# santi-pdp/segan_pytorch

Hardware: AMD Instinct MI355X
Metric: 16384-sample waveform chunks/sec (GAN step) (higher is better)
Workload: dtype f32

## Files before the change

### include/segan_hip.h

```cpp
#ifndef SEGAN_HIP_H
#define SEGAN_HIP_H

#include <stddef.h>
#include <stdint.h>

#ifdef __cplusplus
extern "C" {
#endif

#define SEGAN_ABI_VERSION 16

#define SEGAN_PAD_REFLECT 0
#define SEGAN_PAD_ZERO 1

#define SEGAN_ACT_NONE 0
#define SEGAN_ACT_TANH 1

typedef struct segan_src {
  const float* p0;
  const float* p1;
  int32_t C0;
  int32_t C1;
  const float* scale;
  const float* shift;
  const float* slope;
} segan_src;

int segan_abi_version(void);
const char* segan_last_error(void);

int segan_set_reserved_slots(int n);

size_t segan_packed_f_bytes(int M, int N, int S);
size_t segan_packed_t_bytes(int M, int N, int S);

int segan_pack_weights(const float* w, float* wf, float* wt, int M, int N, int K, int S,
                       int pad_t, void* stream);

#define SEGAN_PREC_FP32 0
#define SEGAN_PREC_BF16 1
#define SEGAN_PREC_BF16X3 3
#define SEGAN_PREC_FP32_BLOCKED 4
size_t segan_packed_bf_bytes(int M, int N, int S, int tform, int planes);
int segan_pack_weights_bf(const float* w, void* out, int M, int N, int K, int S, int tform,
                          int pad_t, int planes, void* stream);

size_t segan_bf16_scratch_bytes(int op, int B, int N, int M, int L, int K, int S, int pad, int planes);
size_t segan_corr_scratch_bytes(void);
void segan_debug_last_corr(int* out6);
void segan_debug_last_wgrad(int* out6);

int segan_conv1d_fwd(const segan_src* x, const void* wf, const float* bias, float* out, int B,
                     int N, int M, int L, int K, int S, int padL, int mode, int roll,
                     int precision, void* scratch, size_t scratch_bytes, void* stream);

int segan_conv1d_dgrad(const float* da, const void* wt, const float* w, float* dx, float* halo,
                       int B, int N, int M, int L, int K, int S, int padL, int roll, int precision,
                       void* scratch, size_t scratch_bytes, void* stream);

#define SEGAN_WGRAD_DETERMINISTIC 1
size_t segan_wgrad_scratch_bytes(int B, int M, int N, int Ls, int S, int precision, int flags);
int segan_wgrad(const segan_src* lo, const segan_src* hi, float* dw, int B, int M, int N, int Ls,
                int K, int S, int padL, int mode, int roll, int precision, int flags, void* scratch,
                size_t scratch_bytes, void* stream);

int segan_deconv1d_fwd(const segan_src* x, const void* wt, const float* w, const float* bias,
                       float* y, int B, int M, int N, int Ls, int K, int S, int pad, int act,
                       int precision, void* scratch, size_t scratch_bytes, void* stream);

int segan_deconv1d_dgrad(const float* dy, const void* wf, float* dx0, float* dx1, int B, int M,
                         int M0, int N, int Ls, int K, int S, int pad, int precision, void* scratch,
                         size_t scratch_bytes, void* stream);


int segan_bn_nsplit(int B, int C, int L);
int segan_bn_stats(const float* x, const float* gamma, const float* beta, float eps,
                   float momentum, float* running_mean, float* running_var, float* mean,
                   float* rstd, float* scale, float* shift, float* ws, int B, int C, int L,
                   void* stream);
int segan_bn_partial(const float* x, float* ws, int B, int C, int L, void* stream);
int segan_bn_final(const float* ws, int nsplit_total, const float* gamma, const float* beta,
                   float eps, float momentum, float* running_mean, float* running_var, float* mean,
                   float* rstd, float* scale, float* shift, int C, void* stream);

int segan_affine_tanh(const float* x, const float* scale, const float* shift, float* y, int B,
                      int C, int L, void* stream);
int segan_scale_mask(const float* x, const float* scale, const float* mask, float* y, int B, int C,
                     int L, void* stream);

int segan_affine_prelu(const float* x, const float* scale, const float* shift, const float* slope,
                       float* y, int B, int C, int L, void* stream);

int segan_sum_skip(const float* x0, const float* slope0, const float* x1, const float* alpha,
                   float* out, int B, int C, int L, void* stream);

int segan_act_bwd(const float* a, const float* dh, const float* dskip, const float* slope,
                  const float* alpha, const float* bn_mean, const float* bn_rstd,
                  const float* bn_gamma, const float* bn_beta, float* da, float* dslope,
                  float* dalpha, float* dgamma, float* dbeta, float* dbias, float* ws, int B, int C,
                  int L, void* stream);
int segan_act_bwd_bn_reduce(const float* a, const float* dh, const float* slope,
                            const float* bn_mean, const float* bn_rstd, const float* bn_gamma,
                            const float* bn_beta, float* dslope, float* dgamma, float* dbeta,
                            float* totals, float* ws, int B, int C, int L, void* stream);
int segan_act_bwd_bn_apply(const float* a, const float* dh, const float* slope,
                           const float* bn_mean, const float* bn_rstd, const float* bn_gamma,
                           const float* bn_beta, const float* totals, float* da, float* dbias,
                           float* ws, int B, int C, int L, double count_total, void* stream);

int segan_tanh_bwd(const float* y, const float* dy, const float* clean, float l1_scale, float* da,
                   float* dbias, float* ws, int B, int C, int L, void* stream);


#define SEGAN_GEMM_DETERMINISTIC 1
size_t segan_gemm_scratch_bytes(int M, int N, int K);
int segan_gemm(const float* A, int64_t sam, int64_t sak, const float* B, int64_t sbk, int64_t sbn,
               float* C, int64_t ldc, int M, int N, int K, int beta0, int flags, void* scratch,
               size_t scratch_bytes, void* stream);

int segan_bias_prelu_rows(const float* x, const float* bias, const float* slope, float* y,
                          int rows, int cols, void* stream);
int segan_bias_prelu_rows_bwd(const float* x, const float* bias, const float* slope,
                              const float* dy, float* dx, float* dslope, float* dbias, int rows,
                              int cols, void* stream);

int segan_mse_const(const float* x, float target, float* loss, float* grad, const float* gout,
                    float gscale, int n, void* stream);
int segan_bce_logits_const(const float* x, float target, float* loss, float* grad,
                           const float* gout, float gscale, int n, void* stream);
int segan_l1_mean(const float* x, const float* y, float* loss, float* ws, int64_t n,
                  void* stream);
int segan_l1_bwd(const float* x, const float* y, const float* gout, float gscale, float* grad,
                 int64_t n, void* stream);

size_t segan_packed_g_bytes(int M, int N, int S);
int segan_pack_weights_g(const float* w, float* wg, int M, int N, int K, int S, void* stream);
int segan_conv1d_dgrad_short(const float* da, const float* wg, float* dx, int B, int N, int M,
                             int L, int K, int S, int padL, int roll, void* stream);

int segan_pool_time_fwd(const float* x, float* y, int* idx, int rows, int L, int mode,
                        void* stream);
int segan_pool_time_bwd(const float* dy, const int* idx, float* dx, int rows, int L, int mode,
                        void* stream);

int segan_mse_mean(const float* x, const float* y, float* loss, float* ws, int64_t n,
                   void* stream);
int segan_mse_bwd(const float* x, const float* y, const float* gout, float gscale, float* grad,
                  int64_t n, void* stream);

size_t segan_snorm_ws_floats(int A, int Bd, int K, int dim);
int segan_snorm_fwd(const float* w, float* u, float* v, float* w_sn, float* sigma, float* ws, int A,
                    int Bd, int K, int dim, int power_iteration, float eps, void* stream);
int segan_snorm_bwd(const float* dw_sn, const float* w, const float* u, const float* v,
                    const float* sigma, float* dw, float* ws, int A, int Bd, int K, int dim,
                    void* stream);

int segan_stft_pitch(int n_fft);
int segan_stft_basis(float* basis, int n_fft, int win, void* stream);
int segan_stft_frames(const float* x, float* frames, int B, int T, int n_fft, int hop, int win,
                      void* stream);
int segan_powdb(const float* S, float* db, int64_t rows, int nbins, int pitch, float eps,
                void* stream);
int segan_powdb_bwd(const float* S, const float* ddb, float* dS, int64_t rows, int nbins, int pitch,
                    float eps, void* stream);
int segan_stft_overlap_add(const float* dframes, float* dx, int B, int T, int n_fft, int hop,
                           int win, void* stream);

int segan_pcm16_prep(const int16_t* pcm, const unsigned char* first, float* clean, float* noisy,
                     int B, int T, double coef, void* stream);

int segan_deemphasis(const float* y, float* x, int rows, int T, double coef, void* stream);
int segan_ssnr_frames(int T, int srate);
int segan_ssnr(const float* ref, const float* deg, float* seg, float* out, int rows, int T,
               int srate, double eps, void* stream);
int segan_wss(const float* ref, const float* deg, double* dist, int rows, int T, int srate,
              void* stream);
int segan_llr(const float* ref, const float* deg, double* dist, int rows, int T, int srate,
              void* stream);
int segan_stoi_plan(int srate, int* pq, int* ntaps, double* taps, int cap, int* bands);
int segan_stoi_dims(int T, int srate, int* dims);
int segan_stoi(const float* ref, const float* deg, const int* lengths, int rows, int T, int srate,
               double* xr, double* yr, double* energy, int* mask, int* kept, int* count,
               double* xs, double* ys, double* X, double* Y, double* rho, double* d, void* stream);

int segan_rmsprop_step(float* p, const float* g, float* sq, float lr, float alpha, float eps,
                       int64_t n, void* stream);
int segan_adam_step(float* p, const float* g, float* m, float* v, float lr, double beta1,
                    double beta2, float eps, int step, int64_t n, void* stream);
int segan_fill(float* p, float value, int64_t n, void* stream);
int segan_scale(float* p, float s, int64_t n, void* stream);

int segan_comm_id_bytes(void);
int segan_comm_unique_id(void* id_out);
int segan_comm_init(void** comm_out, int world, int rank, const void* id);
int segan_comm_destroy(void* comm);
int segan_comm_rank(void* comm);
int segan_comm_world(void* comm);
int segan_allreduce(void* comm, float* buf, size_t n, float scale, void* stream);
int segan_broadcast(void* comm, float* buf, size_t n, int root, void* stream);
int segan_allgather(void* comm, const float* send, float* recv, size_t n, void* stream);

#ifdef __cplusplus
}
#endif
#endif
```

### segan_pytorch_amd/_lib.py

```python
import ctypes
import os
from ctypes import POINTER, Structure, c_char_p, c_double, c_float, c_int, c_int32, c_int64, c_size_t, c_void_p

_HERE = os.path.dirname(os.path.abspath(__file__))
LIB_PATH = os.environ.get('SEGAN_HIP_LIB') or os.path.join(_HERE, 'libsegan_hip.so')

PAD_REFLECT = 0
PAD_ZERO = 1
ACT_NONE = 0
ACT_TANH = 1
ABI_VERSION = 16


class SeganSrc(Structure):
    _fields_ = [('p0', c_void_p), ('p1', c_void_p), ('C0', c_int32), ('C1', c_int32),
                ('scale', c_void_p), ('shift', c_void_p), ('slope', c_void_p)]


_P = c_void_p
_SRC = POINTER(SeganSrc)

SIGNATURES = {
    'segan_abi_version': (c_int, []),
    'segan_set_reserved_slots': (c_int, [c_int]),
    'segan_last_error': (c_char_p, []),
    'segan_packed_f_bytes': (c_size_t, [c_int, c_int, c_int]),
    'segan_packed_t_bytes': (c_size_t, [c_int, c_int, c_int]),
    'segan_pack_weights': (c_int, [_P, _P, _P, c_int, c_int, c_int, c_int, c_int, _P]),
    'segan_packed_bf_bytes': (c_size_t, [c_int, c_int, c_int, c_int, c_int]),
    'segan_pack_weights_bf': (c_int, [_P, _P, c_int, c_int, c_int, c_int, c_int, c_int, c_int, _P]),
    'segan_corr_scratch_bytes': (c_size_t, []),
    'segan_bf16_scratch_bytes': (c_size_t, [c_int] * 9),
    'segan_debug_last_corr': (None, [POINTER(c_int)]),
    'segan_debug_last_wgrad': (None, [POINTER(c_int)]),
    'segan_conv1d_fwd': (c_int, [_SRC, _P, _P, _P, c_int, c_int, c_int, c_int, c_int, c_int, c_int,
                                 c_int, c_int, c_int, _P, c_size_t, _P]),
    'segan_conv1d_dgrad': (c_int, [_P, _P, _P, _P, _P, c_int, c_int, c_int, c_int, c_int, c_int, c_int,
                                   c_int, c_int, _P, c_size_t, _P]),
    'segan_wgrad': (c_int, [_SRC, _SRC, _P, c_int, c_int, c_int, c_int, c_int, c_int, c_int, c_int,
                            c_int, c_int, c_int, _P, c_size_t, _P]),
    'segan_wgrad_scratch_bytes': (c_size_t, [c_int, c_int, c_int, c_int, c_int, c_int, c_int]),
    'segan_deconv1d_fwd': (c_int, [_SRC, _P, _P, _P, _P, c_int, c_int, c_int, c_int, c_int, c_int, c_int,
                                   c_int, c_int, _P, c_size_t, _P]),
    'segan_deconv1d_dgrad': (c_int, [_P, _P, _P, _P, c_int, c_int, c_int, c_int, c_int, c_int, c_int,
                                     c_int, c_int, _P, c_size_t, _P]),
    'segan_bn_nsplit': (c_int, [c_int, c_int, c_int]),
    'segan_bn_stats': (c_int, [_P, _P, _P, c_float, c_float, _P, _P, _P, _P, _P, _P, _P, c_int, c_int,
                               c_int, _P]),
    'segan_bn_partial': (c_int, [_P, _P, c_int, c_int, c_int, _P]),
    'segan_bn_final': (c_int, [_P, c_int, _P, _P, c_float, c_float, _P, _P, _P, _P, _P, _P, c_int, _P]),
    'segan_act_bwd_bn_reduce': (c_int, [_P] * 12 + [c_int, c_int, c_int, _P]),
    'segan_act_bwd_bn_apply': (c_int, [_P] * 11 + [c_int, c_int, c_int, c_double, _P]),
    'segan_affine_prelu': (c_int, [_P, _P, _P, _P, _P, c_int, c_int, c_int, _P]),
    'segan_affine_tanh': (c_int, [_P, _P, _P, _P, c_int, c_int, c_int, _P]),
    'segan_scale_mask': (c_int, [_P, _P, _P, _P, c_int, c_int, c_int, _P]),
    'segan_sum_skip': (c_int, [_P, _P, _P, _P, _P, c_int, c_int, c_int, _P]),
    'segan_bce_logits_const': (c_int, [_P, c_float, _P, _P, _P, c_float, c_int, _P]),
    'segan_act_bwd': (c_int, [_P] * 16 + [c_int, c_int, c_int, _P]),
    'segan_tanh_bwd': (c_int, [_P, _P, _P, c_float, _P, _P, _P, c_int, c_int, c_int, _P]),
    'segan_gemm_scratch_bytes': (c_size_t, [c_int, c_int, c_int]),
    'segan_gemm': (c_int, [_P, c_int64, c_int64, _P, c_int64, c_int64, _P, c_int64, c_int, c_int,
                           c_int, c_int, c_int, _P, c_size_t, _P]),
    'segan_bias_prelu_rows': (c_int, [_P, _P, _P, _P, c_int, c_int, _P]),
    'segan_bias_prelu_rows_bwd': (c_int, [_P, _P, _P, _P, _P, _P, _P, c_int, c_int, _P]),
    'segan_mse_const': (c_int, [_P, c_float, _P, _P, _P, c_float, c_int, _P]),
    'segan_l1_bwd': (c_int, [_P, _P, _P, c_float, _P, c_int64, _P]),
    'segan_l1_mean': (c_int, [_P, _P, _P, _P, c_int64, _P]),
    'segan_packed_g_bytes': (c_size_t, [c_int, c_int, c_int]),
    'segan_pack_weights_g': (c_int, [_P, _P, c_int, c_int, c_int, c_int, _P]),
    'segan_conv1d_dgrad_short': (c_int, [_P, _P, _P, c_int, c_int, c_int, c_int, c_int, c_int, c_int,
                                        c_int, _P]),
    'segan_pool_time_fwd': (c_int, [_P, _P, _P, c_int, c_int, c_int, _P]),
    'segan_pool_time_bwd': (c_int, [_P, _P, _P, c_int, c_int, c_int, _P]),
    'segan_mse_mean': (c_int, [_P, _P, _P, _P, c_int64, _P]),
    'segan_mse_bwd': (c_int, [_P, _P, _P, c_float, _P, c_int64, _P]),
    'segan_snorm_ws_floats': (c_size_t, [c_int, c_int, c_int, c_int]),
    'segan_snorm_fwd': (c_int, [_P, _P, _P, _P, _P, _P, c_int, c_int, c_int, c_int, c_int, c_float, _P]),
    'segan_snorm_bwd': (c_int, [_P, _P, _P, _P, _P, _P, _P, c_int, c_int, c_int, c_int, _P]),
    'segan_pcm16_prep': (c_int, [_P, _P, _P, _P, c_int, c_int, c_double, _P]),
    'segan_stft_basis': (c_int, [_P, c_int, c_int, _P]),
    'segan_stft_frames': (c_int, [_P, _P, c_int, c_int, c_int, c_int, c_int, _P]),
    'segan_stft_pitch': (c_int, [c_int]),
    'segan_powdb': (c_int, [_P, _P, c_int64, c_int, c_int, c_float, _P]),
    'segan_powdb_bwd': (c_int, [_P, _P, _P, c_int64, c_int, c_int, c_float, _P]),
    'segan_stft_overlap_add': (c_int, [_P, _P, c_int, c_int, c_int, c_int, c_int, _P]),
    'segan_deemphasis': (c_int, [_P, _P, c_int, c_int, c_double, _P]),
    'segan_ssnr_frames': (c_int, [c_int, c_int]),
    'segan_ssnr': (c_int, [_P, _P, _P, _P, c_int, c_int, c_int, c_double, _P]),
    'segan_wss': (c_int, [_P, _P, _P, c_int, c_int, c_int, _P]),
    'segan_llr': (c_int, [_P, _P, _P, c_int, c_int, c_int, _P]),
    'segan_stoi_plan': (c_int, [c_int, POINTER(c_int), POINTER(c_int), _P, c_int, POINTER(c_int)]),
    'segan_stoi_dims': (c_int, [c_int, c_int, POINTER(c_int)]),
    'segan_stoi': (c_int, [_P, _P, _P, c_int, c_int, c_int] + [_P] * 13),
    'segan_rmsprop_step': (c_int, [_P, _P, _P, c_float, c_float, c_float, c_int64, _P]),
    'segan_adam_step': (c_int, [_P, _P, _P, _P, c_float, c_double, c_double, c_float, c_int, c_int64,
                                _P]),
    'segan_fill': (c_int, [_P, c_float, c_int64, _P]),
    'segan_scale': (c_int, [_P, c_float, c_int64, _P]),
    'segan_comm_id_bytes': (c_int, []),
    'segan_comm_unique_id': (c_int, [_P]),
    'segan_comm_init': (c_int, [POINTER(c_void_p), c_int, c_int, _P]),
    'segan_comm_destroy': (c_int, [_P]),
    'segan_comm_rank': (c_int, [_P]),
    'segan_comm_world': (c_int, [_P]),
    'segan_allreduce': (c_int, [_P, _P, c_size_t, c_float, _P]),
    'segan_broadcast': (c_int, [_P, _P, c_size_t, c_int, _P]),
    'segan_allgather': (c_int, [_P, _P, _P, c_size_t, _P]),
}

_lib = None


def load():
    global _lib
    if _lib is not None:
        return _lib
    if not os.path.exists(LIB_PATH):
        raise RuntimeError(
            'segan_pytorch_amd: {} not found. Build it with `make` (or '
            '`python -c "import __graft_entry__ as g; g.build()"`) at the repo root. '
            'There is no non-HIP fallback.'.format(LIB_PATH))
    try:
        import torch
        if torch.cuda.is_available():
            torch.cuda.init()
    except ImportError:
        pass
    lib = ctypes.CDLL(LIB_PATH)
    for name, (res, args) in SIGNATURES.items():
        fn = getattr(lib, name)
        fn.restype = res
        fn.argtypes = args
    ver = lib.segan_abi_version()
    if ver != ABI_VERSION:
        raise RuntimeError('libsegan_hip ABI {} != expected {}'.format(ver, ABI_VERSION))
    _lib = lib
    return lib


def check(rc, what=''):
    if rc != 0:
        msg = load().segan_last_error()
        raise RuntimeError('libsegan_hip {} failed ({}): {}'.format(
            what, rc, msg.decode() if msg else '?'))
```

### segan_pytorch_amd/csrc/segan_conv.hip

```cpp
#include "segan_conv_shared.h"

template <int MB, int NB, int WM, int U>
struct TileGeom {
  static constexpr int S = 32 / U;
  static constexpr int WN = 4 / WM;
  static constexpr int NI = MB / (32 * WM);
  static constexpr int NJ = NB / (32 * WN);
  static constexpr int NPT = MB / S;
};

struct TileWork {
  int tile, c0, c1;
  bool partial;
  int piece;
};

struct TileIter {
  int tileA;
  long unit, unit_end;
  int first_tile;
  __device__ __forceinline__ void init(const CorrArgs& a, int nch) {
    tileA = blockIdx.x;
    unit = (long)blockIdx.x * a.sk_units;
    unit_end = min(unit + (long)a.sk_units, a.sk_total);
// ... 882 lines not shown
    const int row = (int)(t / hl), j = (int)(t - (long)row * hl);
    const int P = j < padL ? j : L + j;
    const int idx = segan_hi_index(P, L, padL, SEGAN_PAD_REFLECT, roll);
    if (idx >= 0) dx[(size_t)row * L + idx] += halo[(size_t)row * hl + j];
    return;
  }
  const int row = blockIdx.x * blockDim.x + threadIdx.x;
  if (row >= rows) return;
  float* d = dx + (size_t)row * L;
  const float* hrow = halo + (size_t)row * hl;
  for (int P = 0; P < padL; ++P) {
    const int idx = segan_hi_index(P, L, padL, SEGAN_PAD_REFLECT, roll);
    if (idx >= 0) d[idx] += hrow[P];
  }
  for (int P2 = 0; P2 < padR; ++P2) {
    const int idx = segan_hi_index(L + padL + P2, L, padL, SEGAN_PAD_REFLECT, roll);
    if (idx >= 0) d[idx] += hrow[padL + P2];
  }
}

#define CS_KC 16
struct ShortArgs {
  const float* da;
  const float* wg;
  float* dx;
  int B, N, M, L, Ls, padL, padRw, roll, ncoltiles;
  int xr8, xbc;
};

template <int S>
__global__ __launch_bounds__(256, 2) void conv_dgrad_short_kernel(const ShortArgs a) {
  constexpr int MB = 128, NB = 128, KC = CS_KC, NI = 2, NJ = 2, YP = 65, U = 32 / S;
  extern __shared__ __attribute__((aligned(16))) float smem[];
  float* Wl0 = smem;
  float* Il0 = smem + 2 * KC * MB;
  const int tid = threadIdx.x;
  const int lane = tid & 63;
  const int wave = __builtin_amdgcn_readfirstlane(tid >> 6);
  const int wm = wave >> 1, wn = wave & 1;
  const int l31 = lane & 31, h = lane >> 5;
  int rowtile, coltile;
  if (a.xbc > 0) {
    const int x = blockIdx.x & 7, k = blockIdx.x >> 3;
    const int per = a.xr8 * a.xbc;
    const int cb = k / per, rem = k - cb * per;
    const int wdt = min(a.xbc, a.ncoltiles - cb * a.xbc);
    const int rr = rem / wdt;
    rowtile = x * a.xr8 + rr;
    coltile = cb * a.xbc + rem - rr * wdt;
  } else {
    const int vb = xcd_remap(blockIdx.x, gridDim.x);
    rowtile = vb / a.ncoltiles;
    coltile = vb - rowtile * a.ncoltiles;
  }
  const int Ls = a.Ls, L = a.L;
  const int n0 = rowtile * 4;
  const int b0 = coltile * (NB / Ls);
  const int rowpitch = a.N * 32;

  const long wbytes = (long)a.M * rowpitch * 4, xbytes = (long)a.B * a.M * Ls * 4;
  const __amdgpu_buffer_rsrc_t wrs = __builtin_amdgcn_make_buffer_rsrc(
      const_cast<float*>(a.wg), 0, (int)(wbytes < 0x7fffffffL ? wbytes : 0x7fffffffL), 0x00020000);
  const __amdgpu_buffer_rsrc_t xrs = __builtin_amdgcn_make_buffer_rsrc(
      const_cast<float*>(a.da), 0, (int)(xbytes < 0x7fffffffL ? xbytes : 0x7fffffffL), 0x00020000);
  const int lr = lane >> 5, lc = 4 * (lane & 31);
  const int wvo = (lr * rowpitch + rowtile * MB + lc) * 4;
  const int s_l = lc / Ls, t_l = lc - s_l * Ls;
  const int xvo = (b0 + s_l < a.B) ? ((s_l * a.M + lr) * Ls + t_l) * 4 : (int)0x80000000u;

  auto load_chunk = [&](int ch, int buf) {
    float* Wl = Wl0 + buf * (KC * MB);
    float* Il = Il0 + buf * (KC * NB);
#pragma unroll
    for (int p = 0; p < KC / 8; ++p) {
      const int q = wave + 4 * p;
      __builtin_amdgcn_raw_ptr_buffer_load_lds(
          wrs, (__attribute__((address_space(3))) void*)(Wl + q * 256), 16, wvo,
          (ch * KC + 2 * q) * rowpitch * 4, 0, 0);
      __builtin_amdgcn_raw_ptr_buffer_load_lds(
          xrs, (__attribute__((address_space(3))) void*)(Il + q * 256), 16, xvo,
          ((b0 * a.M + ch * KC + 2 * q) * Ls) * 4, 0, 0);
    }
  };

  int aoff[NI], boff[NJ], rsh[NI];
#pragma unroll
  for (int i = 0; i < NI; ++i) {
    aoff[i] = h * MB + 32 * (wm * NI + i) + l31;
    rsh[i] = 0;
  }
#pragma unroll
  for (int j = 0; j < NJ; ++j) boff[j] = h * NB + 64 * wn + 32 * j + l31;

  f32x16 acc[NI][NJ];
#pragma unroll
  for (int i = 0; i < NI; ++i)
#pragma unroll
    for (int j = 0; j < NJ; ++j)
#pragma unroll
      for (int e = 0; e < 16; ++e) acc[i][j][e] = 0.0f;

  const int nch = a.M / KC;
  float b30_unused[NJ] = {};
  load_chunk(0, 0);
  __builtin_amdgcn_s_waitcnt(0x0f70);
  __syncthreads();
  for (int ch = 0; ch < nch; ++ch) {
    const int buf = ch & 1;
    if (ch + 1 < nch) load_chunk(ch + 1, buf ^ 1);
    corr_mma_chunk<MB, 1, KC, NI, NJ, false>(Wl0 + buf * (KC * MB), Il0 + buf * (KC * NB), NB, aoff,
                                             boff, rsh, acc, b30_unused, h, aoff, boff);
    __builtin_amdgcn_s_waitcnt(0x0f70);
    __syncthreads();
  }

  float* Yb = smem + wave * (32 * YP);
  const int bw = b0 + (64 * wn) / Ls;
  auto dxp = [&](int P, int cbase) -> float {
    const int r = P % S, qq = P / S;
    float v = 0.0f;
#pragma unroll
    for (int u = 0; u < U; ++u) {
      const int t = qq - u;
      if (t >= 0 && t < Ls) v += Yb[(r * U + u) * YP + cbase + t];
    }
    return v;
  };
#pragma unroll
  for (int i = 0; i < NI; ++i) {
#pragma unroll
    for (int j = 0; j < NJ; ++j)
#pragma unroll
      for (int e = 0; e < 16; ++e)
        Yb[((e & 3) + 8 * (e >> 2) + 4 * h) * YP + 32 * j + l31] = acc[i][j][e];
    __syncthreads();
    const int n = n0 + 2 * wm + i;
#pragma unroll
    for (int p = 0; p < S; ++p) {
      const int o = p * 64 + lane;
      const int sl = o / L, io = o - sl * L;
      const int b = bw + sl;
      float v = dxp(io + a.padL, sl * Ls);
      if (io >= 1 && io <= a.padL) v += dxp(a.padL - io, sl * Ls);
      const int jr = L - 2 - io;
      if (jr >= 0 && jr < a.padRw) v += dxp(L + a.padL + jr, sl * Ls);
      if (b < a.B && n < a.N) {
        int ii = io - a.roll;
        if (ii < 0) ii += L;
        if (ii >= L) ii -= L;
        a.dx[((size_t)b * a.N + n) * L + ii] = v;
      }
    }
    __syncthreads();
  }
}

__global__ void pack_g_kernel(const float* __restrict__ w, float* __restrict__ wg, int M, int N,
                              int K, int S) {
  const size_t total = (size_t)M * N * 32;
  const int U = 32 / S;
  for (size_t i = blockIdx.x * (size_t)blockDim.x + threadIdx.x; i < total;
       i += (size_t)gridDim.x * blockDim.x) {
    const int c = (int)(i & 31);
    const size_t mn = i >> 5;
    const int k = S * (c % U) + c / U;
    wg[i] = k < K ? w[mn * K + k] : 0.0f;
  }
}

static thread_local int g_last_corr[6];
void segan_note_corr_launch(int kind, unsigned grid, const CorrArgs& a, int ntiles) {
  g_last_corr[0] = kind;
  g_last_corr[1] = (int)grid;
  g_last_corr[2] = ntiles;
  g_last_corr[3] = a.sk_nfull;
  g_last_corr[4] = a.sk_total > 0 ? a.sk_units : 0;
  g_last_corr[5] = a.xf_mode;
}
extern "C" void segan_debug_last_corr(int* out6) {
  for (int i = 0; i < 6; ++i) out6[i] = g_last_corr[i];
}

static int cur_device() {
  int d = 0;
  (void)hipGetDevice(&d);
  return d & 15;
}

template <typename K>
static void allow_big_lds(K kern, bool (&done)[16]) {
  const int d = cur_device();
  if (!done[d]) {
    (void)hipFuncSetAttribute(reinterpret_cast<const void*>(kern),
                              hipFuncAttributeMaxDynamicSharedMemorySize, 160 * 1024);
    done[d] = true;
  }
}

template <typename K>
static int resident_per_cu(K kern, size_t lds, int (&occ)[16], size_t (&occ_lds)[16]) {
  const int d = cur_device();
  if (occ[d] == 0 || occ_lds[d] != lds) {
    int nb = 0;
    if (hipOccupancyMaxActiveBlocksPerMultiprocessor(&nb, reinterpret_cast<const void*>(kern), 256,
                                                     lds) != hipSuccess || nb < 1)
      nb = 2;
    occ[d] = nb > 4 ? 4 : nb;
    occ_lds[d] = lds;
  }
  return occ[d];
}

static unsigned plan_streamk(CorrArgs& a, int ntiles, int nch, int occ, size_t slab_floats,
                             bool allow, bool pair_cuts = false) {
  a.sk_nfull = ntiles;
  a.sk_units = 1;
  a.sk_total = 0;
  const double classic_eff = (double)ntiles / (256.0 * ceil_div(ntiles, 256));
  if (!allow || a.act != SEGAN_ACT_NONE || ntiles < 64 || nch < 8 || classic_eff >= 0.97) {
    if (allow && a.act == SEGAN_ACT_NONE && ntiles >= 2 * 256 * occ) return (unsigned)segan_grid_slots(occ);
    return (unsigned)ntiles;
  }
  const int G = segan_grid_slots(occ);
  if (a.sk_ws == nullptr || a.sk_ws_floats < (size_t)G * 2 * slab_floats) return (unsigned)ntiles;
  a.sk_nfull = (ntiles / G) * G;
  const int rem = ntiles - a.sk_nfull;
  if (rem == 0) return (unsigned)ntiles;
  a.sk_total = (long)rem * nch;
  a.sk_units = (int)((a.sk_total + G - 1) / G);
  if (pair_cuts) a.sk_units += a.sk_units & 1;
  return (unsigned)G;
}

template <int MB, int NB, int WM, int U, bool IN_HI, bool OUT_HI, bool SHIFT, int MAXPOS, int KC>
static int launch_corr_t(CorrArgs a, hipStream_t st, bool allow_sk) {
  constexpr int CV = KC / U;
  constexpr int S = 32 / U;
  const int nrowtiles = OUT_HI ? a.NP / (MB / S) : ceil_div(a.Rvalid, MB);
  const size_t lds = (size_t)(2 * KC * MB + 2 * CV * a.RLs) * sizeof(float);
  if (lds > 160 * 1024) {
    segan_set_error("corr: LDS tile %zu B too large (RLs=%d)", lds, a.RLs);
    return SEGAN_EUNSUPPORTED;
  }
  auto kern = corr_kernel<MB, NB, WM, U, IN_HI, OUT_HI, SHIFT, MAXPOS, KC>;
  static bool attr_done[16];
  static int occ[16];
  static size_t occ_lds[16];
  allow_big_lds(kern, attr_done);
  a.rt0 = (!OUT_HI && a.out0 == nullptr) ? a.OC0 / MB : 0;
  const int ntiles = (nrowtiles - a.rt0) * a.ncoltiles;
  const int nch = ceil_div(a.Ktot, KC);
  const unsigned grid = plan_streamk(a, ntiles, nch, resident_per_cu(kern, lds, occ, occ_lds),
                                     (size_t)MB * NB, allow_sk);
  segan_note_corr_launch(1, grid, a, ntiles);
  hipLaunchKernelGGL(kern, dim3(grid), dim3(256), lds, st, a);
  if (int e = segan_check_launch("corr_kernel")) return e;
  if (a.sk_total > 0) {
    hipLaunchKernelGGL((corr_fixup_kernel<MB, NB, WM, U, OUT_HI, KC>), dim3(ntiles - a.sk_nfull),
                       dim3(256), 0, st, a);
    return segan_check_launch("corr_fixup_kernel");
  }
  return SEGAN_OK;
}

template <int MB, int NB, int WM, int U, bool IN_HI, bool OUT_HI, bool SHIFT, bool XF, bool BLK = false>
static int launch_corr2_x(CorrArgs a, hipStream_t st, bool allow_sk) {
  constexpr int KC = CORR2_KC;
  constexpr int CV = KC / U;
  constexpr int S = 32 / U;
  constexpr int SL = 4 / CV;
  const int nrowtiles = OUT_HI ? ceil_div(a.Nout, MB / S) : ceil_div(a.Rvalid, MB);
  a.RLv = a.RLs;
  a.RLs = round_up(a.RLs, 64 * SL);
  a.nld = a.RLs / (64 * SL);
  const size_t lds = (size_t)(2 * KC * MB + 2 * CV * a.RLs) * sizeof(float);
  auto kern = corr2_kernel<MB, NB, WM, U, IN_HI, OUT_HI, SHIFT, XF, BLK>;
  static bool attr_done[16];
  static int occ[16];
  static size_t occ_lds[16];
  allow_big_lds(kern, attr_done);
  a.rt0 = (!OUT_HI && a.out0 == nullptr) ? a.OC0 / MB : 0;
  const int ntiles = (nrowtiles - a.rt0) * a.ncoltiles;
  const int nch = ceil_div(a.Ktot, KC);
  const unsigned grid = plan_streamk(a, ntiles, nch, resident_per_cu(kern, lds, occ, occ_lds),
                                     (size_t)MB * NB, allow_sk, a.f_pair != 0);
  SEGAN_REQUIRE(!a.f_pair || ((nch & 1) == 0 && (a.sk_total == 0 || (a.sk_units & 1) == 0)),
                "corr2: paired channels need even pieces (nch=%d, sk_units=%d)", nch, a.sk_units);
  segan_note_corr_launch(2, grid, a, ntiles);
  hipLaunchKernelGGL(kern, dim3(grid), dim3(256), lds, st, a);
  if (int e = segan_check_launch("corr2_kernel")) return e;
  if (a.sk_total > 0) {
    hipLaunchKernelGGL((corr_fixup_kernel<MB, NB, WM, U, OUT_HI, KC>), dim3(ntiles - a.sk_nfull),
                       dim3(256), 0, st, a);
    return segan_check_launch("corr_fixup_kernel");
  }
  return SEGAN_OK;
}

template <int MB, int NB, int WM, int U, bool IN_HI, bool OUT_HI, bool SHIFT>
static int launch_corr2_t(CorrArgs& a, hipStream_t st, bool allow_sk) {
  if constexpr (U == 8 && MB == 128) {
    if (a.acc_block)
      return a.xf_mode ? launch_corr2_x<MB, NB, WM, U, IN_HI, OUT_HI, SHIFT, true, true>(a, st, allow_sk)
                       : launch_corr2_x<MB, NB, WM, U, IN_HI, OUT_HI, SHIFT, false, true>(a, st, allow_sk);
  }
  return a.xf_mode ? launch_corr2_x<MB, NB, WM, U, IN_HI, OUT_HI, SHIFT, true>(a, st, allow_sk)
                   : launch_corr2_x<MB, NB, WM, U, IN_HI, OUT_HI, SHIFT, false>(a, st, allow_sk);
}

template <int U>
static bool corr2_ok(const CorrArgs& a, int NB) {
  constexpr int SL = 4 / (CORR2_KC / U);
  if (a.RLs > 64 * SL * CORR2_NLD) return false;
  if (a.mode == SEGAN_PAD_ZERO && a.xf_mode == 2) return false;
  if (a.in.C1 > 0 && a.in.C0 != a.in.C1 && samples_per_tile(a.Tcols, NB) > 1) return false;
  return true;
}

template <int U>
// ... 174 lines not shown
                                    int precision, void* scratch, size_t scratch_bytes,
                                    void* stream) {
  const int acc_block = precision == SEGAN_PREC_FP32_BLOCKED;
  if (acc_block) precision = SEGAN_PREC_FP32;
  SEGAN_REQUIRE(precision_ok(precision), "deconv1d_dgrad: precision must be 0, 1, 3 or 4");
  SEGAN_REQUIRE(stride_ok(S), "deconv1d_dgrad: stride %d not in {1,2,4}", S);
  SEGAN_REQUIRE(K >= 1 && K <= 32, "deconv1d_dgrad: kernel width %d not in [1,32]", K);
  SEGAN_REQUIRE(B > 0 && N > 0 && M > 0 && Ls > 0, "deconv1d_dgrad: bad sizes");
  SEGAN_REQUIRE(M0 >= 0 && M0 <= M, "deconv1d_dgrad: split %d outside [0,%d]", M0, M);
  SEGAN_REQUIRE(dy && wf, "deconv1d_dgrad: NULL pointer");
  SEGAN_REQUIRE(dx0 || dx1, "deconv1d_dgrad: both destinations NULL");
  const int U = 32 / S;
  CorrArgs a = {};
  a.acc_block = acc_block;
  a.in.p0 = dy; a.in.p1 = nullptr; a.in.C0 = N; a.in.C1 = 0;
  a.in.scale = a.in.shift = a.in.slope = nullptr;
  a.wp = (const float*)wf;
  a.bias = nullptr; a.halo = nullptr;
  a.B = B; a.Cv = N * S; a.Ktot = N * 32; a.RP = f_pitch(M); a.Rvalid = M;
  a.Tcols = Ls; a.Ctot = B * Ls;
  a.Lin = S * Ls; a.padL = pad; a.mode = SEGAN_PAD_ZERO; a.roll = 0;
  a.win_start = 0; a.H = U - 1;
  a.NP = 1; a.Nout = 0;
  if (M0 == 0) { a.out0 = dx1; a.OC0 = M; a.out1 = nullptr; a.OC1 = 0; }
  else { a.out0 = dx0; a.OC0 = M0; a.out1 = dx1; a.OC1 = M - M0; }
  a.Lout = Ls; a.act = SEGAN_ACT_NONE;
  a.out0_elems = (size_t)B * a.OC0 * Ls;
  a.out1_elems = (size_t)B * a.OC1 * Ls;
  a.f_pair = f_pair(N, K); a.zphase = -1;
  if (precision) {
    CorrArgs a2 = a;
    const int e = segan_corr_bf2_f(a2, U, wf, precision, scratch, scratch_bytes, (hipStream_t)stream);
    return e;
  }
  set_scratch(a, scratch, scratch_bytes);
  return launch_corr<true, false>(a, U, (hipStream_t)stream);
}

extern "C" int segan_deconv1d_fwd(const segan_src* x, const void* wt, const float* w,
                                  const float* bias, float* y, int B, int M, int N, int Ls, int K,
                                  int S, int pad, int act, int precision, void* scratch,
                                  size_t scratch_bytes, void* stream) {
  const int acc_block = precision == SEGAN_PREC_FP32_BLOCKED;
  if (acc_block) precision = SEGAN_PREC_FP32;
  SEGAN_REQUIRE(precision_ok(precision), "deconv1d_fwd: precision must be 0, 1, 3 or 4");
  SEGAN_REQUIRE(stride_ok(S), "deconv1d_fwd: stride %d not in {1,2,4}", S);
  SEGAN_REQUIRE(K >= 1 && K <= 32, "deconv1d_fwd: kernel width %d not in [1,32]", K);
  SEGAN_REQUIRE(B > 0 && N > 0 && M > 0 && Ls > 0, "deconv1d_fwd: bad sizes");
  SEGAN_REQUIRE(y && (wt || (w && N <= 2)), "deconv1d_fwd: NULL pointer");
  SEGAN_REQUIRE(pad >= 0 && K - 2 * pad - S == (K & 1),
                "deconv1d_fwd: K=%d S=%d pad=%d does not give an output of S*Ls samples", K, S, pad);
  SEGAN_REQUIRE(act == SEGAN_ACT_NONE || act == SEGAN_ACT_TANH, "deconv1d_fwd: bad activation");
  if (int e = check_src(x, M, "deconv1d_fwd")) return e;
  const int U = 32 / S;
  CorrArgs a = {};
  a.acc_block = acc_block;
  a.in = *x;
  a.wp = (const float*)wt;
  a.out0 = y; a.out1 = nullptr; a.bias = bias; a.halo = nullptr;
  a.NP = t_np(N, S); a.Nout = N;
  a.B = B; a.Cv = M; a.Ktot = M * U; a.RP = t_pitch(N, S); a.Rvalid = S * a.NP;
  a.Tcols = Ls; a.Ctot = B * Ls;
  a.Lin = Ls; a.padL = 0; a.mode = SEGAN_PAD_ZERO; a.roll = 0;
  int cmin = 1 << 30, cmax = 0;
  for (int r = 0; r < S; ++r) {
    const int c = (r + pad) / S;
    cmin = c < cmin ? c : cmin;
    cmax = c > cmax ? c : cmax;
  }
  for (int r = 0; r < 4; ++r) a.rowshift[r] = r < S ? (r + pad) / S - cmin : 0;
  a.win_start = cmin - (U - 1);
  a.H = U - 1 + (cmax - cmin);
  a.OC0 = N; a.OC1 = 0; a.Lout = S * Ls; a.act = act;
  a.o_padL = 0; a.o_roll = 0; a.o_padR = 0;
  a.out0_elems = (size_t)B * N * S * Ls;
  a.f_pair = 0; a.zphase = t_zphase(K, S, pad);
  if (w && N <= 2) return segan_launch_tsmall(a, w, K, M, N, S, pad, (hipStream_t)stream);
  if (precision && act == SEGAN_ACT_NONE) {
    CorrArgs a2 = a;
    const int e = segan_corr_bf2_t(a2, U, wt, precision, scratch, scratch_bytes, (hipStream_t)stream);
    return e;
  }
  SEGAN_REQUIRE(precision == 0, "deconv1d_fwd: tanh epilogue only on the fp32 path");
  set_scratch(a, scratch, scratch_bytes);
  return launch_corr<false, true>(a, U, (hipStream_t)stream);
}

extern "C" int segan_conv1d_dgrad(const float* da, const void* wt, const float* w, float* dx,
                                  float* halo, int B, int N, int M, int L, int K, int S, int padL,
                                  int roll, int precision, void* scratch, size_t scratch_bytes,
                                  void* stream) {
  const int acc_block = precision == SEGAN_PREC_FP32_BLOCKED;
  if (acc_block) precision = SEGAN_PREC_FP32;
  SEGAN_REQUIRE(precision_ok(precision), "conv1d_dgrad: precision must be 0, 1, 3 or 4");
  SEGAN_REQUIRE(stride_ok(S), "conv1d_dgrad: stride %d not in {1,2,4}", S);
  SEGAN_REQUIRE(K >= 1 && K <= 32, "conv1d_dgrad: kernel width %d not in [1,32]", K);
  SEGAN_REQUIRE(B > 0 && N > 0 && M > 0 && L > 0 && L % S == 0, "conv1d_dgrad: bad sizes");
  SEGAN_REQUIRE(da && dx && halo && (wt || (w && N <= 2)), "conv1d_dgrad: NULL pointer");
  SEGAN_REQUIRE(roll > -L && roll < L, "conv1d_dgrad: |roll| must be < L");
  const int padR = K - 1 - padL >= 0 ? (K - S - padL > 0 ? K - S - padL : 0) : -1;
  SEGAN_REQUIRE(padL >= 0 && padR >= 0 && padL < L && K - S - padL < L, "conv1d_dgrad: bad padding");
  const int U = 32 / S;
  const int Ls = L / S;
  hipStream_t st = (hipStream_t)stream;
  CorrArgs a = {};
  a.acc_block = acc_block;
  a.in.p0 = da; a.in.p1 = nullptr; a.in.C0 = M; a.in.C1 = 0;
  a.in.scale = a.in.shift = a.in.slope = nullptr;
  a.wp = (const float*)wt;
  a.out0 = dx; a.out1 = nullptr; a.bias = nullptr; a.halo = halo;
  a.NP = t_np(N, S); a.Nout = N;
  a.B = B; a.Cv = M; a.Ktot = M * U; a.RP = t_pitch(N, S); a.Rvalid = S * a.NP;
  a.Tcols = (L + padL + padR - 1) / S + 1;
  a.Ctot = B * a.Tcols;
  a.Lin = Ls; a.padL = 0; a.mode = SEGAN_PAD_ZERO; a.roll = 0;
  for (int r = 0; r < 4; ++r) a.rowshift[r] = 0;
  a.win_start = -(U - 1);
  a.H = U - 1;
  a.OC0 = N; a.OC1 = 0; a.Lout = L; a.act = SEGAN_ACT_NONE;
  a.o_padL = padL; a.o_roll = roll; a.o_padR = padR;
  a.out0_elems = (size_t)B * N * L;
  a.halo_elems = (size_t)B * N * (padL + padR);
  a.f_pair = 0; a.zphase = t_zphase(K, S, 0);
  set_scratch(a, scratch, scratch_bytes);
  int e;
  if (w && N <= 2) {
    e = segan_launch_tsmall(a, w, K, M, N, S, 0, st);
  } else if (precision) {
    CorrArgs a2 = a;
    e = segan_corr_bf2_t(a2, U, wt, precision, scratch, scratch_bytes, st);
  } else {
    e = launch_corr<false, true>(a, U, st);
  }
  if (e) return e;
  if (padL + padR > 0) {
    const int rows = B * N;
    const int per_sample = (padL < L - 1 - padR) ? 1 : 0;
    const long nthreads = per_sample ? (long)rows * (padL + padR) : rows;
    hipLaunchKernelGGL(fold_halo_kernel, dim3((unsigned)((nthreads + 255) / 256)), dim3(256), 0, st,
                       dx, halo, rows, L, padL, padR, roll, per_sample);
    return segan_check_launch("fold_halo_kernel");
  }
  return SEGAN_OK;
}

static bool short_ok(int N, int M, int L, int K, int S, int padL) {
  if (!stride_ok(S) || L % S != 0) return false;
  const int Ls = L / S;
  return (Ls == 4 || Ls == 8 || Ls == 16 || Ls == 32 || Ls == 64) && N % 4 == 0 &&
         M % CS_KC == 0 && K >= 1 && K <= 32 && padL >= 0 && K - 1 - padL >= 0 && padL < L &&
         K - S - padL < L;
}

extern "C" size_t segan_packed_g_bytes(int M, int N, int S) {
  if (!stride_ok(S) || M <= 0 || N <= 0) return 0;
  return (size_t)M * N * 32 * sizeof(float);
}

extern "C" int segan_pack_weights_g(const float* w, float* wg, int M, int N, int K, int S,
                                    void* stream) {
  SEGAN_REQUIRE(w && wg && M > 0 && N > 0, "pack_weights_g: bad arguments");
  SEGAN_REQUIRE(stride_ok(S) && K >= 1 && K <= 32, "pack_weights_g: stride in {1,2,4}, K <= 32");
  const size_t total = (size_t)M * N * 32;
  const int blocks = (int)((total + 255) / 256 > 8192 ? 8192 : (total + 255) / 256);
  hipLaunchKernelGGL(pack_g_kernel, dim3(blocks), dim3(256), 0, (hipStream_t)stream, w, wg, M, N, K,
                     S);
  return segan_check_launch("pack_weights_g");
}

extern "C" int segan_conv1d_dgrad_short(const float* da, const float* wg, float* dx, int B, int N,
                                        int M, int L, int K, int S, int padL, int roll,
                                        void* stream) {
  SEGAN_REQUIRE(da && wg && dx && B > 0, "conv1d_dgrad_short: bad arguments");
  SEGAN_REQUIRE(roll > -L && roll < L, "conv1d_dgrad_short: |roll| must be < L");
  if (!short_ok(N, M, L, K, S, padL)) {
    segan_set_error("conv1d_dgrad_short: geometry not covered (L/S in {4,8,16,32,64}, N %% 4 == 0, "
                    "M %% 16 == 0)");
    return SEGAN_EUNSUPPORTED;
  }
  ShortArgs a;
  a.da = da; a.wg = wg; a.dx = dx;
  a.B = B; a.N = N; a.M = M; a.L = L; a.Ls = L / S; a.padL = padL;
  a.padRw = K - S - padL > 0 ? K - S - padL : 0;
  a.roll = roll;
  a.ncoltiles = ceil_div(B, 128 / a.Ls);
  const size_t lds = 4 * 32 * 65 * sizeof(float);
  const dim3 grid((unsigned)(N / 4 * a.ncoltiles));
  static const bool blocked = [] {
    const char* e = getenv("SEGAN_SHORT_ORDER");
    return !(e && e[0] == '0');
  }();
  a.xr8 = a.xbc = 0;
  if (blocked && (N / 4) % 8 == 0) {
    a.xr8 = N / 4 / 8;
    a.xbc = a.xr8 >= 128 ? 1 : 128 / a.xr8;
  }
  hipStream_t st = (hipStream_t)stream;
  if (S == 4) hipLaunchKernelGGL(conv_dgrad_short_kernel<4>, grid, dim3(256), lds, st, a);
  else if (S == 2) hipLaunchKernelGGL(conv_dgrad_short_kernel<2>, grid, dim3(256), lds, st, a);
  else hipLaunchKernelGGL(conv_dgrad_short_kernel<1>, grid, dim3(256), lds, st, a);
  return segan_check_launch("conv_dgrad_short_kernel");
}
```

### segan_pytorch_amd/csrc/segan_pack.hip

```cpp
#include "segan_conv_shared.h"

__global__ __launch_bounds__(256) void pack_f_kernel(const float* __restrict__ w,
                                                     float* __restrict__ wf, int M, int N, int K,
                                                     int S, int U, int pitch, int rows, int pair) {
  __shared__ float t[64][33];
  const int n = blockIdx.y;
  const int m0 = blockIdx.x * 64;
  const int tid = threadIdx.x;
  {
    float v[8];
#pragma unroll
    for (int i = 0; i < 8; ++i) {
      const int e = tid + 256 * i;
      const int ml = e >> 5, k = e & 31;
      const int m = m0 + ml;
      v[i] = (m < M && n < N && k < K) ? w[((size_t)m * N + n) * K + k] : 0.0f;
    }
#pragma unroll
    for (int i = 0; i < 8; ++i) {
      const int e = tid + 256 * i;
      t[e >> 5][e & 31] = v[i];
    }
  }
  __syncthreads();
  if (pair && (n & 1) && n < N && tid < 64) {
    const int m = m0 + tid;
    t[tid][31] = m < M ? w[((size_t)m * N + n - 1) * K + (31 - S)] : 0.0f;
  }
  __syncthreads();
  for (int e = tid; e < 32 * 64; e += 256) {
    const int kk = e >> 6, ml = e & 63;
    const int r = kk / U, u = kk - r * U;
    const int row = (n * S + r) * U + u;
    if (row < rows && m0 + ml < pitch) wf[(size_t)row * pitch + m0 + ml] = t[ml][S * u + r];
  }
}

__global__ __launch_bounds__(256) void pack_t_kernel(const float* __restrict__ w,
                                                     float* __restrict__ wt, int M, int N, int K,
                                                     int S, int U, int NP, int pad, int pitch,
                                                     int rows) {
  __shared__ float t[64][33];
  const int m = blockIdx.y;
  const int n0 = blockIdx.x * 64;
  const int tid = threadIdx.x;
  {
    float v[8];
#pragma unroll
    for (int i = 0; i < 8; ++i) {
      const int e = tid + 256 * i;
      const int nl = e >> 5, k = e & 31;
      const int n = n0 + nl;
      v[i] = (m < M && n < N && k < K) ? w[((size_t)m * N + n) * K + k] : 0.0f;
    }
#pragma unroll
    for (int i = 0; i < 8; ++i) {
      const int e = tid + 256 * i;
      t[e >> 5][e & 31] = v[i];
    }
  }
  __syncthreads();
  for (int e = tid; e < 32 * 64; e += 256) {
    const int kk = e >> 6, nl = e & 63;
    const int up = kk / S, r = kk - up * S;
    const int rho = (r + pad) % S;
    const int k = S * (U - 1 - up) + rho;
    const int row = m * U + up;
    const int n = n0 + nl;
    if (row < rows && n < NP) wt[(size_t)row * pitch + r * NP + n] = t[nl][k];
  }
}

extern "C" size_t segan_packed_f_bytes(int M, int N, int S) {
  if (!stride_ok(S) || M <= 0 || N <= 0) return 0;
  return (size_t)f_rows(N) * f_pitch(M) * sizeof(float);
}
extern "C" size_t segan_packed_t_bytes(int M, int N, int S) {
  if (!stride_ok(S) || M <= 0 || N <= 0) return 0;
  return (size_t)t_rows(M, S) * t_pitch(N, S) * sizeof(float);
}

extern "C" int segan_pack_weights(const float* w, float* wf, float* wt, int M, int N, int K, int S,
                                  int pad_t, void* stream) {
  SEGAN_REQUIRE(w != nullptr, "pack_weights: w is NULL");
  SEGAN_REQUIRE(stride_ok(S), "pack_weights: stride %d not in {1,2,4}", S);
  SEGAN_REQUIRE(K >= 1 && K <= 32, "pack_weights: kernel width %d not in [1,32]", K);
  SEGAN_REQUIRE(M > 0 && N > 0, "pack_weights: bad channel counts %d,%d", M, N);
  SEGAN_REQUIRE(pad_t >= 0, "pack_weights: negative padding");
  hipStream_t st = (hipStream_t)stream;
  const int U = 32 / S;
  if (wf) {
    const int pitch = f_pitch(M), rows = f_rows(N);
    hipLaunchKernelGGL(pack_f_kernel, dim3(pitch / 64, ceil_div(rows, 32)), dim3(256), 0, st, w,
                       wf, M, N, K, S, U, pitch, rows, f_pair(N, K));
  }
  if (wt) {
    const int NP = t_np(N, S);
    const int pitch = t_pitch(N, S), rows = t_rows(M, S);
    hipLaunchKernelGGL(pack_t_kernel, dim3(ceil_div(NP, 64), ceil_div(rows, U)), dim3(256), 0, st,
                       w, wt, M, N, K, S, U, NP, pad_t, pitch, rows);
  }
  return segan_check_launch("pack_weights");
}
```

### segan_pytorch_amd/csrc/segan_pointwise.hip

```cpp
#include "segan_common.h"

#define PW_THREADS 256

static int pw_nsplit(int B, int C, int L) {
  int ns = ceil_div(2048, C);
  if (ns > B) ns = B;
  long per = (long)B * L / ns;
  while (ns > 1 && per < 2048) {
    ns = (ns + 1) / 2;
    per = (long)B * L / ns;
  }
  return ns < 1 ? 1 : ns;
}

extern "C" int segan_bn_nsplit(int B, int C, int L) {
  if (B <= 0 || C <= 0 || L <= 0) return 0;
  return pw_nsplit(B, C, L);
}

template <int NV>
__device__ __forceinline__ void block_sum(float (&v)[NV], float* sm) {
  const int lane = threadIdx.x & 63, wave = threadIdx.x >> 6;
#pragma unroll
  for (int k = 0; k < NV; ++k) v[k] = warp_sum(v[k]);
  if (lane == 0)
#pragma unroll
    for (int k = 0; k < NV; ++k) sm[wave * NV + k] = v[k];
  __syncthreads();
  if (threadIdx.x == 0) {
#pragma unroll
    for (int k = 0; k < NV; ++k) {
      float s = 0.f;
      for (int w = 0; w < PW_THREADS / 64; ++w) s += sm[w * NV + k];
      v[k] = s;
    }
  }
  __syncthreads();
}

struct ChanRange {
  int c, b_beg, b_end;
};
__device__ __forceinline__ ChanRange chan_range(int B, int nsplit) {
  ChanRange r;
  r.c = blockIdx.x;
  const int per = (B + nsplit - 1) / nsplit;
  r.b_beg = blockIdx.y * per;
  r.b_end = min(B, r.b_beg + per);
  return r;
}

__device__ __forceinline__ void chan_combine(float& n, float& mean, float& m2, float nb, float mb,
                                             float qb) {
  const float tot = n + nb;
  if (tot <= 0.0f) return;
  const float d = mb - mean;
  const float f = nb / tot;
  mean = fmaf(d, f, mean);
  m2 = m2 + qb + d * d * n * f;
  n = tot;
}

__global__ void bn_partial_kernel(const float* __restrict__ x, float* __restrict__ ws, int B, int C,
                                  int L, int nsplit) {
  __shared__ float sm[3 * (PW_THREADS / 64)];
  const ChanRange cr = chan_range(B, nsplit);
  const int nb = cr.b_end - cr.b_beg;
  const float* base = x + ((size_t)cr.b_beg * C + cr.c) * L;
  const size_t sstride = (size_t)C * L;
  const bool vec = (L & 3) == 0 && ((uintptr_t)x & 15) == 0;
  const int Lv = vec ? L >> 2 : L;
  int tr = PW_THREADS;
  while (tr > Lv && tr > 1) tr >>= 1;
  const int rp = PW_THREADS / tr;
  const int t0 = threadIdx.x % tr, r0 = threadIdx.x / tr;
  float K = 0.0f, s1 = 0.0f, s2 = 0.0f, n = 0.0f;
  if (r0 < nb && t0 < Lv) K = base[(size_t)r0 * sstride + (vec ? 4 * t0 : t0)];
  for (int b = r0; b < nb; b += rp) {
    const float* row = base + b * sstride;
    if (vec) {
      for (int t = t0; t < Lv; t += tr) {
        const f32x4 u = *reinterpret_cast<const f32x4*>(row + 4 * t);
#pragma unroll
        for (int e = 0; e < 4; ++e) {
          const float d = u[e] - K;
          s1 += d;
          s2 = fmaf(d, d, s2);
        }
        n += 4.0f;
      }
    } else {
      for (int t = t0; t < Lv; t += tr) {
        const float d = row[t] - K;
        s1 += d;
        s2 = fmaf(d, d, s2);
        n += 1.0f;
      }
    }
  }
  float mean = 0.0f, m2 = 0.0f;
  if (n > 0.0f) {
    const float r = s1 / n;
    mean = K + r;
    m2 = fmaxf(s2 - s1 * r, 0.0f);
  }
#pragma unroll
  for (int o = 32; o > 0; o >>= 1) {
    const float nb2 = __shfl_down(n, o, 64), mb2 = __shfl_down(mean, o, 64), qb2 = __shfl_down(m2, o, 64);
    chan_combine(n, mean, m2, nb2, mb2, qb2);
  }
  const int lane = threadIdx.x & 63, wave = threadIdx.x >> 6;
  if (lane == 0) {
    sm[3 * wave] = n; sm[3 * wave + 1] = mean; sm[3 * wave + 2] = m2;
  }
  __syncthreads();
  if (threadIdx.x == 0) {
    for (int w = 1; w < PW_THREADS / 64; ++w) chan_combine(n, mean, m2, sm[3 * w], sm[3 * w + 1], sm[3 * w + 2]);
    float* w = ws + ((size_t)blockIdx.y * C + cr.c) * 3;
    w[0] = n;
    w[1] = mean;
    w[2] = m2;
  }
}

__device__ __forceinline__ void bn_affine(float gamma, float beta, float mean, float rstd,
                                          float& scale, float& shift) {
  scale = gamma * rstd;
  shift = fmaf(-mean, scale, beta);
}

__global__ void bn_final_kernel(const float* __restrict__ ws, const float* gamma, const float* beta,
                                float eps, float momentum, float* running_mean, float* running_var,
                                float* mean_o, float* rstd_o, float* scale_o, float* shift_o, int C,
                                int nsplit) {
  const int c = blockIdx.x * blockDim.x + threadIdx.x;
  if (c >= C) return;
  double n = 0.0, mean = 0.0, m2 = 0.0;
  for (int s = 0; s < nsplit; ++s) {
    const float* w = ws + ((size_t)s * C + c) * 3;
    const double nb = w[0], mb = w[1], qb = w[2];
    if (nb <= 0.0) continue;
    const double tot = n + nb;
    const double d = mb - mean;
    mean += d * nb / tot;
    m2 += qb + d * d * n * nb / tot;
    n = tot;
  }
  const double var = n > 0 ? m2 / n : 0.0;
  const float rstd = (float)(1.0 / sqrt(var + (double)eps));
  const float g = gamma ? gamma[c] : 1.0f;
  const float bt = beta ? beta[c] : 0.0f;
  float sc, sh;
  bn_affine(g, bt, (float)mean, rstd, sc, sh);
  if (mean_o) mean_o[c] = (float)mean;
  if (rstd_o) rstd_o[c] = rstd;
  if (scale_o) scale_o[c] = sc;
  if (shift_o) shift_o[c] = sh;
  if (running_mean) running_mean[c] = (1.0f - momentum) * running_mean[c] + momentum * (float)mean;
  if (running_var) {
    const double unb = n > 1 ? m2 / (n - 1.0) : var;
    running_var[c] = (1.0f - momentum) * running_var[c] + momentum * (float)unb;
  }
}

extern "C" int segan_bn_stats(const float* x, const float* gamma, const float* beta, float eps,
                              float momentum, float* running_mean, float* running_var, float* mean,
                              float* rstd, float* scale, float* shift, float* ws, int B, int C,
                              int L, void* stream) {
  SEGAN_REQUIRE(x && ws, "bn_stats: NULL pointer");
  SEGAN_REQUIRE(B > 0 && C > 0 && L > 0, "bn_stats: bad sizes");
  hipStream_t st = (hipStream_t)stream;
  const int ns = pw_nsplit(B, C, L);
  hipLaunchKernelGGL(bn_partial_kernel, dim3(C, ns), dim3(PW_THREADS), 0, st, x, ws, B, C, L, ns);
  hipLaunchKernelGGL(bn_final_kernel, dim3(ceil_div(C, 64)), dim3(64), 0, st, ws, gamma, beta, eps,
                     momentum, running_mean, running_var, mean, rstd, scale, shift, C, ns);
  return segan_check_launch("bn_stats");
}

extern "C" int segan_bn_partial(const float* x, float* ws, int B, int C, int L, void* stream) {
  SEGAN_REQUIRE(x && ws, "bn_partial: NULL pointer");
  SEGAN_REQUIRE(B > 0 && C > 0 && L > 0, "bn_partial: bad sizes");
  const int ns = pw_nsplit(B, C, L);
  hipLaunchKernelGGL(bn_partial_kernel, dim3(C, ns), dim3(PW_THREADS), 0, (hipStream_t)stream, x, ws,
                     B, C, L, ns);
  return segan_check_launch("bn_partial");
}

extern "C" int segan_bn_final(const float* ws, int nsplit_total, const float* gamma,
                              const float* beta, float eps, float momentum, float* running_mean,
                              float* running_var, float* mean, float* rstd, float* scale,
                              float* shift, int C, void* stream) {
  SEGAN_REQUIRE(ws && nsplit_total > 0 && C > 0, "bn_final: bad arguments");
  hipLaunchKernelGGL(bn_final_kernel, dim3(ceil_div(C, 64)), dim3(64), 0, (hipStream_t)stream, ws,
                     gamma, beta, eps, momentum, running_mean, running_var, mean, rstd, scale, shift,
                     C, nsplit_total);
  return segan_check_launch("bn_final");
}

__global__ void affine_prelu_kernel(const float* __restrict__ x, const float* scale,
                                    const float* shift, const float* slope, float* __restrict__ y,
                                    size_t total, int C, int L) {
  for (size_t i = blockIdx.x * (size_t)blockDim.x + threadIdx.x; i < total;
       i += (size_t)gridDim.x * blockDim.x) {
    const int c = (int)((i / L) % C);
    float v = x[i];
    v = fmaf(v, scale ? scale[c] : 1.0f, shift ? shift[c] : 0.0f);
    if (slope) v = v > 0.f ? v : v * slope[c];
    y[i] = v;
  }
}

extern "C" int segan_affine_prelu(const float* x, const float* scale, const float* shift,
                                  const float* slope, float* y, int B, int C, int L, void* stream) {
  SEGAN_REQUIRE(x && y, "affine_prelu: NULL pointer");
  SEGAN_REQUIRE(B > 0 && C > 0 && L > 0, "affine_prelu: bad sizes");
  const size_t total = (size_t)B * C * L;
  const int blocks = (int)((total + 255) / 256 > 4096 ? 4096 : (total + 255) / 256);
  hipLaunchKernelGGL(affine_prelu_kernel, dim3(blocks), dim3(256), 0, (hipStream_t)stream, x, scale,
                     shift, slope, y, total, C, L);
  return segan_check_launch("affine_prelu");
}

__global__ void affine_tanh_kernel(const float* __restrict__ x, const float* scale,
                                   const float* shift, float* __restrict__ y, size_t total, int C,
                                   int L) {
  for (size_t i = blockIdx.x * (size_t)blockDim.x + threadIdx.x; i < total;
       i += (size_t)gridDim.x * blockDim.x) {
    const int c = (int)((i / L) % C);
    y[i] = tanhf(fmaf(x[i], scale ? scale[c] : 1.0f, shift ? shift[c] : 0.0f));
  }
}

extern "C" int segan_affine_tanh(const float* x, const float* scale, const float* shift, float* y,
                                 int B, int C, int L, void* stream) {
  SEGAN_REQUIRE(x && y, "affine_tanh: NULL pointer");
  SEGAN_REQUIRE(B > 0 && C > 0 && L > 0, "affine_tanh: bad sizes");
  const size_t total = (size_t)B * C * L;
  const int blocks = (int)((total + 255) / 256 > 4096 ? 4096 : (total + 255) / 256);
  hipLaunchKernelGGL(affine_tanh_kernel, dim3(blocks), dim3(256), 0, (hipStream_t)stream, x, scale,
                     shift, y, total, C, L);
  return segan_check_launch("affine_tanh");
}

__global__ void scale_mask_kernel(const float* __restrict__ x, const float* scale,
                                  const float* __restrict__ mask, float* __restrict__ y,
                                  size_t total, int C, int L) {
  for (size_t i = blockIdx.x * (size_t)blockDim.x + threadIdx.x; i < total;
       i += (size_t)gridDim.x * blockDim.x) {
    const int c = (int)((i / L) % C);
    y[i] = x[i] * (scale ? scale[c] : 1.0f) * mask[i];
  }
}

extern "C" int segan_scale_mask(const float* x, const float* scale, const float* mask, float* y,
                                int B, int C, int L, void* stream) {
  SEGAN_REQUIRE(x && mask && y, "scale_mask: NULL pointer");
  SEGAN_REQUIRE(B > 0 && C > 0 && L > 0, "scale_mask: bad sizes");
  const size_t total = (size_t)B * C * L;
  const int blocks = (int)((total + 255) / 256 > 4096 ? 4096 : (total + 255) / 256);
  hipLaunchKernelGGL(scale_mask_kernel, dim3(blocks), dim3(256), 0, (hipStream_t)stream, x, scale,
                     mask, y, total, C, L);
  return segan_check_launch("scale_mask");
}

__global__ void sum_skip_kernel(const float* __restrict__ x0, const float* slope0,
                                const float* __restrict__ x1, const float* alpha,
                                float* __restrict__ out, size_t total, int C, int L) {
  for (size_t i = blockIdx.x * (size_t)blockDim.x + threadIdx.x; i < total;
       i += (size_t)gridDim.x * blockDim.x) {
    const int c = (int)((i / L) % C);
    float v = x0[i];
    if (slope0) v = v > 0.f ? v : v * slope0[c];
    out[i] = fmaf(alpha[c], x1[i], v);
  }
}

extern "C" int segan_sum_skip(const float* x0, const float* slope0, const float* x1,
                              const float* alpha, float* out, int B, int C, int L, void* stream) {
  SEGAN_REQUIRE(x0 && x1 && alpha && out, "sum_skip: NULL pointer");
  SEGAN_REQUIRE(B > 0 && C > 0 && L > 0, "sum_skip: bad sizes");
  const size_t total = (size_t)B * C * L;
  const int blocks = (int)((total + 255) / 256 > 4096 ? 4096 : (total + 255) / 256);
  hipLaunchKernelGGL(sum_skip_kernel, dim3(blocks), dim3(256), 0, (hipStream_t)stream, x0, slope0,
                     x1, alpha, out, total, C, L);
  return segan_check_launch("sum_skip");
}

struct ActBwdArgs {
  const float* a;
  const float* dh;
  const float* dskip;
  const float* slope;
  const float* alpha;
  const float* mean;
  const float* rstd;
  const float* gamma;
  const float* beta;
  float* da;
  float* ws;
  int B, C, L, nsplit;
  float inv_count;
};

template <int PHASE>
__global__ void act_bwd_kernel(const ActBwdArgs p) {
  __shared__ float sm[16];
  const ChanRange cr = chan_range(p.B, p.nsplit);
  const int c = cr.c;
  const int nb = cr.b_end - cr.b_beg;
  const float sl = p.slope ? p.slope[c] : 1.0f;
  const float al = p.alpha ? p.alpha[c] : 0.0f;
  float mu = 0.f, rs = 1.f, ga = 1.f, be = 0.f, dbeta_m = 0.f, dgamma_m = 0.f, sc = 1.f, sh = 0.f;
  if (PHASE != 0) {
    mu = p.mean[c];
    rs = p.rstd[c];
    ga = p.gamma ? p.gamma[c] : 1.0f;
    be = p.beta ? p.beta[c] : 0.0f;
    bn_affine(ga, be, mu, rs, sc, sh);
  }
  if (PHASE == 2) {
    const float* tot = p.ws + (size_t)p.nsplit * p.C * 4 + (size_t)c * 2;
    dbeta_m = tot[0] * p.inv_count;
    dgamma_m = tot[1] * p.inv_count;
  }
  float r[3] = {0.f, 0.f, 0.f};
  const bool has_skip = p.dskip != nullptr;
  auto elem = [&](float av, float dh, float ds) -> float {
    if (PHASE == 0) {
      float g = dh * (av > 0.f ? 1.0f : sl);
      r[0] += dh * (av > 0.f ? 0.0f : av);
      if (has_skip) {
        g = fmaf(al, ds, g);
        r[1] = fmaf(ds, av, r[1]);
      }
      r[2] += g;
      return g;
    }
    const float xh = (av - mu) * rs;
    const float v = fmaf(av, sc, sh);
    const float g = dh * (v > 0.f ? 1.0f : sl);
    if (PHASE == 1) {
      r[0] += dh * (v > 0.f ? 0.0f : v);
      r[1] += g;
      r[2] = fmaf(g, xh, r[2]);
      return 0.0f;
    }
    const float d = ga * rs * (g - dbeta_m - xh * dgamma_m);
    r[0] += d;
    return d;
  };
  const size_t base = ((size_t)cr.b_beg * p.C + c) * p.L;
  const size_t sstride = (size_t)p.C * p.L;
  const bool vec = (p.L & 3) == 0 &&
                   (((uintptr_t)p.a | (uintptr_t)p.dh | (uintptr_t)p.dskip | (uintptr_t)p.da) & 15) == 0;
  const int Lv = vec ? p.L >> 2 : p.L;
  int tr = PW_THREADS;
  while (tr > Lv && tr > 1) tr >>= 1;
  const int rp = PW_THREADS / tr;
  const int t0 = threadIdx.x % tr, r0 = threadIdx.x / tr;
  const f32x4 z4 = {0.f, 0.f, 0.f, 0.f};
  for (int b = r0; b < nb; b += rp) {
    const size_t ro = base + b * sstride;
    if (vec) {
      for (int t = t0; t < Lv; t += tr) {
        const size_t i = ro + 4 * (size_t)t;
        const f32x4 av = *reinterpret_cast<const f32x4*>(p.a + i);
        const f32x4 dh = p.dh ? *reinterpret_cast<const f32x4*>(p.dh + i) : z4;
        const f32x4 ds = has_skip ? *reinterpret_cast<const f32x4*>(p.dskip + i) : z4;
        f32x4 o;
#pragma unroll
        for (int e = 0; e < 4; ++e) o[e] = elem(av[e], dh[e], ds[e]);
        if (PHASE != 1) *reinterpret_cast<f32x4*>(p.da + i) = o;
      }
    } else {
      for (int t = t0; t < Lv; t += tr) {
        const size_t i = ro + t;
        const float o = elem(p.a[i], p.dh ? p.dh[i] : 0.0f, has_skip ? p.dskip[i] : 0.0f);
        if (PHASE != 1) p.da[i] = o;
      }
    }
  }
  block_sum<3>(r, sm);
  if (threadIdx.x == 0) {
    float* w = p.ws + ((size_t)blockIdx.y * p.C + c) * 4;
    w[0] = r[0];
    w[1] = r[1];
    w[2] = r[2];
  }
}

template <int PHASE>
__global__ void act_bwd_final_kernel(const ActBwdArgs p, float* dslope, float* dalpha,
                                     float* dgamma, float* dbeta, float* dbias) {
  const int c = blockIdx.x * blockDim.x + threadIdx.x;
  if (c >= p.C) return;
  float s0 = 0.f, s1 = 0.f, s2 = 0.f;
  for (int s = 0; s < p.nsplit; ++s) {
    const float* w = p.ws + ((size_t)s * p.C + c) * 4;
    s0 += w[0];
    s1 += w[1];
    s2 += w[2];
  }
  if (PHASE == 0) {
    if (dslope) dslope[c] += s0;
    if (dalpha) dalpha[c] += s1;
    if (dbias) dbias[c] += s2;
  } else if (PHASE == 1) {
    if (dslope) dslope[c] += s0;
    if (dbeta) dbeta[c] += s1;
    if (dgamma) dgamma[c] += s2;
    float* tot = p.ws + (size_t)p.nsplit * p.C * 4 + (size_t)c * 2;
    tot[0] = s1;
    tot[1] = s2;
  } else {
    if (dbias) dbias[c] += s0;
  }
}

extern "C" int segan_act_bwd(const float* a, const float* dh, const float* dskip,
                             const float* slope, const float* alpha, const float* bn_mean,
                             const float* bn_rstd, const float* bn_gamma, const float* bn_beta,
                             float* da, float* dslope, float* dalpha, float* dgamma, float* dbeta,
                             float* dbias, float* ws, int B, int C, int L, void* stream) {
  SEGAN_REQUIRE(a && da && ws, "act_bwd: NULL pointer");
  SEGAN_REQUIRE(dh || dskip, "act_bwd: no incoming gradient");
  SEGAN_REQUIRE(B > 0 && C > 0 && L > 0, "act_bwd: bad sizes");
  SEGAN_REQUIRE((bn_mean == nullptr) == (bn_rstd == nullptr), "act_bwd: mean/rstd must pair");
  SEGAN_REQUIRE(!(dskip && !alpha), "act_bwd: dskip needs alpha");
  SEGAN_REQUIRE(!(bn_mean && dskip), "act_bwd: BN layers have no skip tap");
  hipStream_t st = (hipStream_t)stream;
  ActBwdArgs p;
  p.a = a; p.dh = dh; p.dskip = dskip; p.slope = slope; p.alpha = alpha;
  p.mean = bn_mean; p.rstd = bn_rstd; p.gamma = bn_gamma; p.beta = bn_beta;
  p.da = da; p.ws = ws; p.B = B; p.C = C; p.L = L;
  p.nsplit = pw_nsplit(B, C, L);
  p.inv_count = 1.0f / ((float)B * (float)L);
  const dim3 grid(C, p.nsplit), fgrid(ceil_div(C, 64));
  if (!bn_mean) {
    hipLaunchKernelGGL(act_bwd_kernel<0>, grid, dim3(PW_THREADS), 0, st, p);
    hipLaunchKernelGGL(act_bwd_final_kernel<0>, fgrid, dim3(64), 0, st, p, dslope, dalpha, dgamma,
                       dbeta, dbias);
  } else {
    hipLaunchKernelGGL(act_bwd_kernel<1>, grid, dim3(PW_THREADS), 0, st, p);
    hipLaunchKernelGGL(act_bwd_final_kernel<1>, fgrid, dim3(64), 0, st, p, dslope, dalpha, dgamma,
                       dbeta, dbias);
    hipLaunchKernelGGL(act_bwd_kernel<2>, grid, dim3(PW_THREADS), 0, st, p);
    hipLaunchKernelGGL(act_bwd_final_kernel<2>, fgrid, dim3(64), 0, st, p, dslope, dalpha, dgamma,
                       dbeta, dbias);
  }
  return segan_check_launch("act_bwd");
}

extern "C" int segan_act_bwd_bn_reduce(const float* a, const float* dh, const float* slope,
                                       const float* bn_mean, const float* bn_rstd,
                                       const float* bn_gamma, const float* bn_beta, float* dslope,
                                       float* dgamma, float* dbeta, float* totals, float* ws, int B,
                                       int C, int L, void* stream) {
  SEGAN_REQUIRE(a && dh && bn_mean && bn_rstd && totals && ws, "act_bwd_bn_reduce: NULL pointer");
  SEGAN_REQUIRE(B > 0 && C > 0 && L > 0, "act_bwd_bn_reduce: bad sizes");
  hipStream_t st = (hipStream_t)stream;
  ActBwdArgs p;
  p.a = a; p.dh = dh; p.dskip = nullptr; p.slope = slope; p.alpha = nullptr;
  p.mean = bn_mean; p.rstd = bn_rstd; p.gamma = bn_gamma; p.beta = bn_beta;
  p.da = nullptr; p.ws = ws; p.B = B; p.C = C; p.L = L;
  p.nsplit = pw_nsplit(B, C, L);
  p.inv_count = 1.0f / ((float)B * (float)L);
  hipLaunchKernelGGL(act_bwd_kernel<1>, dim3(C, p.nsplit), dim3(PW_THREADS), 0, st, p);
  hipLaunchKernelGGL(act_bwd_final_kernel<1>, dim3(ceil_div(C, 64)), dim3(64), 0, st, p, dslope,
                     (float*)nullptr, dgamma, dbeta, (float*)nullptr);
  if (hipMemcpyAsync(totals, ws + (size_t)p.nsplit * C * 4, (size_t)C * 2 * sizeof(float),
                     hipMemcpyDeviceToDevice, st) != hipSuccess) {
    segan_set_error("act_bwd_bn_reduce: copy of the totals failed");
    return SEGAN_ELAUNCH;
  }
  return segan_check_launch("act_bwd_bn_reduce");
}

extern "C" int segan_act_bwd_bn_apply(const float* a, const float* dh, const float* slope,
                                      const float* bn_mean, const float* bn_rstd,
                                      const float* bn_gamma, const float* bn_beta,
                                      const float* totals, float* da, float* dbias, float* ws, int B,
                                      int C, int L, double count_total, void* stream) {
  SEGAN_REQUIRE(a && dh && bn_mean && bn_rstd && totals && da && ws, "act_bwd_bn_apply: NULL pointer");
  SEGAN_REQUIRE(B > 0 && C > 0 && L > 0 && count_total >= (double)B * L, "act_bwd_bn_apply: bad sizes");
  hipStream_t st = (hipStream_t)stream;
  ActBwdArgs p;
  p.a = a; p.dh = dh; p.dskip = nullptr; p.slope = slope; p.alpha = nullptr;
  p.mean = bn_mean; p.rstd = bn_rstd; p.gamma = bn_gamma; p.beta = bn_beta;
  p.da = da; p.ws = ws; p.B = B; p.C = C; p.L = L;
  p.nsplit = pw_nsplit(B, C, L);
  p.inv_count = (float)(1.0 / count_total);
  if (hipMemcpyAsync(ws + (size_t)p.nsplit * C * 4, totals, (size_t)C * 2 * sizeof(float),
                     hipMemcpyDeviceToDevice, st) != hipSuccess) {
    segan_set_error("act_bwd_bn_apply: copy of the totals failed");
    return SEGAN_ELAUNCH;
  }
  hipLaunchKernelGGL(act_bwd_kernel<2>, dim3(C, p.nsplit), dim3(PW_THREADS), 0, st, p);
  hipLaunchKernelGGL(act_bwd_final_kernel<2>, dim3(ceil_div(C, 64)), dim3(64), 0, st, p,
                     (float*)nullptr, (float*)nullptr, (float*)nullptr, (float*)nullptr, dbias);
  return segan_check_launch("act_bwd_bn_apply");
}

__global__ void tanh_bwd_kernel(const float* __restrict__ y, const float* dy, const float* clean,
                                float l1_scale, float* __restrict__ da, float* ws, int B, int C,
                                int L, int nsplit) {
  __shared__ float sm[16];
  const ChanRange cr = chan_range(B, nsplit);
  const int nb = cr.b_end - cr.b_beg;
  const long cnt = (long)(nb > 0 ? nb : 0) * L;
  float r[1] = {0.f};
  for (long e = threadIdx.x; e < cnt; e += PW_THREADS) {
    const int b = cr.b_beg + (int)(e / L);
    const int t = (int)(e % L);
    const size_t i = ((size_t)b * C + cr.c) * L + t;
    const float yv = y[i];
    float g = dy ? dy[i] : 0.0f;
    if (clean) {
      const float d = yv - clean[i];
      g += l1_scale * (d > 0.f ? 1.0f : (d < 0.f ? -1.0f : 0.0f));
    }
    const float d = g * (1.0f - yv * yv);
    da[i] = d;
    r[0] += d;
  }
  block_sum<1>(r, sm);
  if (threadIdx.x == 0) ws[(size_t)blockIdx.y * C + cr.c] = r[0];
}

__global__ void sum_splits_add_kernel(const float* ws, float* out, int C, int nsplit) {
  const int c = blockIdx.x * blockDim.x + threadIdx.x;
  if (c >= C) return;
  float s = 0.f;
  for (int k = 0; k < nsplit; ++k) s += ws[(size_t)k * C + c];
  out[c] += s;
}

extern "C" int segan_tanh_bwd(const float* y, const float* dy, const float* clean, float l1_scale,
                              float* da, float* dbias, float* ws, int B, int C, int L,
                              void* stream) {
  SEGAN_REQUIRE(y && da && ws, "tanh_bwd: NULL pointer");
  SEGAN_REQUIRE(dy || clean, "tanh_bwd: no incoming gradient");
  SEGAN_REQUIRE(B > 0 && C > 0 && L > 0, "tanh_bwd: bad sizes");
  hipStream_t st = (hipStream_t)stream;
  const int ns = pw_nsplit(B, C, L);
  hipLaunchKernelGGL(tanh_bwd_kernel, dim3(C, ns), dim3(PW_THREADS), 0, st, y, dy, clean, l1_scale,
                     da, ws, B, C, L, ns);
  if (dbias)
    hipLaunchKernelGGL(sum_splits_add_kernel, dim3(ceil_div(C, 64)), dim3(64), 0, st, ws, dbias, C,
                       ns);
  return segan_check_launch("tanh_bwd");
}

__global__ void bias_prelu_rows_kernel(const float* __restrict__ x, const float* bias,
                                       const float* slope, float* __restrict__ y, int rows,
                                       int cols) {
  const size_t total = (size_t)rows * cols;
  for (size_t i = blockIdx.x * (size_t)blockDim.x + threadIdx.x; i < total;
       i += (size_t)gridDim.x * blockDim.x) {
    const int c = (int)(i % cols);
    float v = x[i] + (bias ? bias[c] : 0.0f);
    if (slope) v = v > 0.f ? v : v * slope[c];
    y[i] = v;
  }
}

extern "C" int segan_bias_prelu_rows(const float* x, const float* bias, const float* slope,
                                     float* y, int rows, int cols, void* stream) {
  SEGAN_REQUIRE(x && y && rows > 0 && cols > 0, "bias_prelu_rows: bad arguments");
  const size_t total = (size_t)rows * cols;
  const int blocks = (int)((total + 255) / 256 > 2048 ? 2048 : (total + 255) / 256);
  hipLaunchKernelGGL(bias_prelu_rows_kernel, dim3(blocks), dim3(256), 0, (hipStream_t)stream, x,
                     bias, slope, y, rows, cols);
  return segan_check_launch("bias_prelu_rows");
}

__global__ __launch_bounds__(256) void bias_prelu_rows_bwd_kernel(
    const float* __restrict__ x, const float* bias, const float* slope,
    const float* __restrict__ dy, float* __restrict__ dx, float* dslope, float* dbias, int rows,
    int cols) {
  __shared__ float sm[2][4][64];
  const int cl = threadIdx.x & 63, rg = threadIdx.x >> 6;
  const int c = blockIdx.x * 64 + cl;
  float s_sl = 0.f, s_b = 0.f;
  if (c < cols) {
    const float bs = bias ? bias[c] : 0.0f;
    const float sl = slope ? slope[c] : 1.0f;
    for (int r = rg; r < rows; r += 4) {
      const size_t i = (size_t)r * cols + c;
      const float v = x[i] + bs;
      const float g = dy[i];
      const float d = g * (v > 0.f ? 1.0f : sl);
      s_sl += g * (v > 0.f ? 0.0f : v);
      s_b += d;
      dx[i] = d;
    }
  }
  sm[0][rg][cl] = s_sl;
  sm[1][rg][cl] = s_b;
  __syncthreads();
  if (rg == 0 && c < cols) {
    const float a = sm[0][0][cl] + sm[0][1][cl] + sm[0][2][cl] + sm[0][3][cl];
    const float b = sm[1][0][cl] + sm[1][1][cl] + sm[1][2][cl] + sm[1][3][cl];
    if (dslope && slope) dslope[c] += a;
    if (dbias) dbias[c] += b;
  }
}

extern "C" int segan_bias_prelu_rows_bwd(const float* x, const float* bias, const float* slope,
                                         const float* dy, float* dx, float* dslope, float* dbias,
                                         int rows, int cols, void* stream) {
  SEGAN_REQUIRE(x && dy && dx && rows > 0 && cols > 0, "bias_prelu_rows_bwd: bad arguments");
  hipLaunchKernelGGL(bias_prelu_rows_bwd_kernel, dim3(ceil_div(cols, 64)), dim3(256), 0,
                     (hipStream_t)stream, x, bias, slope, dy, dx, dslope, dbias, rows, cols);
  return segan_check_launch("bias_prelu_rows_bwd");
}

__global__ void mse_const_kernel(const float* __restrict__ x, float target, float* loss,
                                 float* grad, const float* gout, float gscale, int n) {
  __shared__ float sm[16];
  float r[1] = {0.f};
  const float inv = 1.0f / (float)n;
  if (gout) gscale *= gout[0];
  for (int i = threadIdx.x; i < n; i += PW_THREADS) {
    const float d = x[i] - target;
    r[0] = fmaf(d, d, r[0]);
    if (grad) grad[i] = 2.0f * d * inv * gscale;
  }
  block_sum<1>(r, sm);
  if (threadIdx.x == 0 && loss) loss[0] = r[0] * inv;
}

extern "C" int segan_mse_const(const float* x, float target, float* loss, float* grad,
                               const float* gout, float gscale, int n, void* stream) {
  SEGAN_REQUIRE(x && n > 0 && (loss || grad), "mse_const: bad arguments");
  hipLaunchKernelGGL(mse_const_kernel, dim3(1), dim3(PW_THREADS), 0, (hipStream_t)stream, x, target,
                     loss, grad, gout, gscale, n);
  return segan_check_launch("mse_const");
}

__global__ void bce_const_kernel(const float* __restrict__ x, float target, float* loss,
                                 float* grad, const float* gout, float gscale, int n) {
  __shared__ float sm[16];
  float r[1] = {0.f};
  const float inv = 1.0f / (float)n;
  if (gout) gscale *= gout[0];
  for (int i = threadIdx.x; i < n; i += PW_THREADS) {
    const float v = x[i];
    r[0] += fmaxf(v, 0.f) - v * target + log1pf(expf(-fabsf(v)));
    if (grad) grad[i] = (1.0f / (1.0f + expf(-v)) - target) * inv * gscale;
  }
  block_sum<1>(r, sm);
  if (threadIdx.x == 0 && loss) loss[0] = r[0] * inv;
}

extern "C" int segan_bce_logits_const(const float* x, float target, float* loss, float* grad,
                                      const float* gout, float gscale, int n, void* stream) {
  SEGAN_REQUIRE(x && n > 0 && (loss || grad), "bce_logits_const: bad arguments");
  hipLaunchKernelGGL(bce_const_kernel, dim3(1), dim3(PW_THREADS), 0, (hipStream_t)stream, x, target,
                     loss, grad, gout, gscale, n);
  return segan_check_launch("bce_logits_const");
}

template <bool SQ>
__global__ void l1_partial_kernel(const float* __restrict__ x, const float* __restrict__ y,
                                  float* ws, size_t n) {
  __shared__ float sm[16];
  float r[1] = {0.f};
  for (size_t i = blockIdx.x * (size_t)blockDim.x + threadIdx.x; i < n;
       i += (size_t)gridDim.x * blockDim.x) {
    const float d = x[i] - y[i];
    r[0] += SQ ? d * d : fabsf(d);
  }
  block_sum<1>(r, sm);
  if (threadIdx.x == 0) ws[blockIdx.x] = r[0];
}
__global__ void l1_final_kernel(const float* ws, float* loss, int nblocks, float inv) {
  __shared__ float sm[16];
  float r[1] = {0.f};
  for (int i = threadIdx.x; i < nblocks; i += PW_THREADS) r[0] += ws[i];
  block_sum<1>(r, sm);
  if (threadIdx.x == 0) loss[0] = r[0] * inv;
}

extern "C" int segan_l1_mean(const float* x, const float* y, float* loss, float* ws, int64_t n,
                             void* stream) {
  SEGAN_REQUIRE(x && y && loss && ws && n > 0, "l1_mean: bad arguments");
  hipStream_t st = (hipStream_t)stream;
  int blocks = (int)((n + 255) / 256 > 1024 ? 1024 : (n + 255) / 256);
  hipLaunchKernelGGL(l1_partial_kernel<false>, dim3(blocks), dim3(PW_THREADS), 0, st, x, y, ws, (size_t)n);
  hipLaunchKernelGGL(l1_final_kernel, dim3(1), dim3(PW_THREADS), 0, st, ws, loss, blocks,
                     1.0f / (float)n);
  return segan_check_launch("l1_mean");
}

extern "C" int segan_mse_mean(const float* x, const float* y, float* loss, float* ws, int64_t n,
                              void* stream) {
  SEGAN_REQUIRE(x && y && loss && ws && n > 0, "mse_mean: bad arguments");
  hipStream_t st = (hipStream_t)stream;
  int blocks = (int)((n + 255) / 256 > 1024 ? 1024 : (n + 255) / 256);
  hipLaunchKernelGGL(l1_partial_kernel<true>, dim3(blocks), dim3(PW_THREADS), 0, st, x, y, ws, (size_t)n);
  hipLaunchKernelGGL(l1_final_kernel, dim3(1), dim3(PW_THREADS), 0, st, ws, loss, blocks,
                     1.0f / (float)n);
  return segan_check_launch("mse_mean");
}

__global__ void mse_bwd_kernel(const float* __restrict__ x, const float* __restrict__ y,
                               const float* gout, float gscale, float* __restrict__ grad, size_t n) {
  const float g = 2.0f * gscale * (gout ? gout[0] : 1.0f) / (float)n;
  for (size_t i = blockIdx.x * (size_t)blockDim.x + threadIdx.x; i < n;
       i += (size_t)gridDim.x * blockDim.x)
    grad[i] = g * (x[i] - y[i]);
}

extern "C" int segan_mse_bwd(const float* x, const float* y, const float* gout, float gscale,
                             float* grad, int64_t n, void* stream) {
  SEGAN_REQUIRE(x && y && grad && n > 0, "mse_bwd: bad arguments");
  int blocks = (int)((n + 255) / 256 > 4096 ? 4096 : (n + 255) / 256);
  hipLaunchKernelGGL(mse_bwd_kernel, dim3(blocks), dim3(256), 0, (hipStream_t)stream, x, y, gout,
                     gscale, grad, (size_t)n);
  return segan_check_launch("mse_bwd");
}

__global__ void l1_bwd_kernel(const float* __restrict__ x, const float* __restrict__ y,
                              const float* gout, float gscale, float* __restrict__ grad, size_t n) {
  const float g = gscale * (gout ? gout[0] : 1.0f) / (float)n;
  for (size_t i = blockIdx.x * (size_t)blockDim.x + threadIdx.x; i < n;
       i += (size_t)gridDim.x * blockDim.x) {
    const float d = x[i] - y[i];
    grad[i] = d > 0.f ? g : (d < 0.f ? -g : 0.0f);
  }
}

extern "C" int segan_l1_bwd(const float* x, const float* y, const float* gout, float gscale,
                            float* grad, int64_t n, void* stream) {
  SEGAN_REQUIRE(x && y && grad && n > 0, "l1_bwd: bad arguments");
  int blocks = (int)((n + 255) / 256 > 4096 ? 4096 : (n + 255) / 256);
  hipLaunchKernelGGL(l1_bwd_kernel, dim3(blocks), dim3(256), 0, (hipStream_t)stream, x, y, gout,
                     gscale, grad, (size_t)n);
  return segan_check_launch("l1_bwd");
}

__global__ void rmsprop_kernel(float* __restrict__ p, const float* __restrict__ g,
                               float* __restrict__ sq, float lr, float alpha, float eps, size_t n) {
  const size_t n4 = n / 4;
  float4* p4 = reinterpret_cast<float4*>(p);
  const float4* g4 = reinterpret_cast<const float4*>(g);
  float4* s4 = reinterpret_cast<float4*>(sq);
// ... 1 lines not shown
  for (size_t i = blockIdx.x * (size_t)blockDim.x + threadIdx.x; i < n4;
       i += (size_t)gridDim.x * blockDim.x) {
    float4 pv = p4[i], gv = g4[i], sv = s4[i];
#define RMS1(f)                                       \
  sv.f = alpha * sv.f + oma * gv.f * gv.f;            \
  pv.f = pv.f - lr * (gv.f / (sqrtf(sv.f) + eps));
    RMS1(x) RMS1(y) RMS1(z) RMS1(w)
#undef RMS1
    p4[i] = pv;
    s4[i] = sv;
  }
  if (blockIdx.x == 0 && threadIdx.x < (n & 3)) {
    const size_t i = n4 * 4 + threadIdx.x;
    const float gv = g[i];
    const float sv = alpha * sq[i] + oma * gv * gv;
    sq[i] = sv;
    p[i] = p[i] - lr * (gv / (sqrtf(sv) + eps));
  }
}

extern "C" int segan_rmsprop_step(float* p, const float* g, float* sq, float lr, float alpha,
                                  float eps, int64_t n, void* stream) {
  SEGAN_REQUIRE(p && g && sq && n > 0, "rmsprop_step: bad arguments");
  SEGAN_REQUIRE(((uintptr_t)p % 16 == 0) && ((uintptr_t)g % 16 == 0) && ((uintptr_t)sq % 16 == 0),
                "rmsprop_step: arenas must be 16-byte aligned");
  int blocks = (int)((n / 4 + 255) / 256 > 2048 ? 2048 : (n / 4 + 255) / 256);
  if (blocks < 1) blocks = 1;
  hipLaunchKernelGGL(rmsprop_kernel, dim3(blocks), dim3(256), 0, (hipStream_t)stream, p, g, sq, lr,
                     alpha, eps, (size_t)n);
  return segan_check_launch("rmsprop_step");
}

__global__ void adam_kernel(float* __restrict__ p, const float* __restrict__ g,
                            float* __restrict__ m, float* __restrict__ v, float step_size,
                            float omb1, float beta2, float omb2, float eps, float inv_sqrt_bc2,
                            size_t n) {
  for (size_t i = blockIdx.x * (size_t)blockDim.x + threadIdx.x; i < n;
       i += (size_t)gridDim.x * blockDim.x) {
    const float gv = g[i];
    const float mv = m[i] + (gv - m[i]) * omb1;
    const float vv = beta2 * v[i] + omb2 * gv * gv;
    m[i] = mv;
    v[i] = vv;
    const float denom = sqrtf(vv) * inv_sqrt_bc2 + eps;
    p[i] = p[i] - step_size * (mv / denom);
  }
}

extern "C" int segan_adam_step(float* p, const float* g, float* m, float* v, float lr,
                               double beta1, double beta2, float eps, int step, int64_t n,
                               void* stream) {
  SEGAN_REQUIRE(p && g && m && v && n > 0 && step >= 1, "adam_step: bad arguments");
  const double bc1 = 1.0 - pow(beta1, (double)step);
  const double bc2 = 1.0 - pow(beta2, (double)step);
  const float step_size = (float)((double)lr / bc1);
  const float inv_sqrt_bc2 = (float)(1.0 / sqrt(bc2));
  int blocks = (int)((n + 255) / 256 > 4096 ? 4096 : (n + 255) / 256);
  hipLaunchKernelGGL(adam_kernel, dim3(blocks), dim3(256), 0, (hipStream_t)stream, p, g, m, v,
                     step_size, (float)(1.0 - beta1), (float)beta2, (float)(1.0 - beta2), eps,
                     inv_sqrt_bc2, (size_t)n);
  return segan_check_launch("adam_step");
}

template <int MODE>
__global__ void pool_time_kernel(const float* __restrict__ x, float* __restrict__ y,
                                 int* __restrict__ idx, int rows, int L) {
  const int lane = threadIdx.x & 63;
  const int row = blockIdx.x * (blockDim.x >> 6) + (threadIdx.x >> 6);
  if (row >= rows) return;
  const float* xr = x + (size_t)row * L;
  if (MODE == 0) {
    float best = -INFINITY;
    int bi = 0x7fffffff;
    for (int t = lane; t < L; t += 64) {
      const float v = xr[t];
      if (v > best || bi == 0x7fffffff) { best = v; bi = t; }
    }
#pragma unroll
    for (int o = 32; o > 0; o >>= 1) {
      const float ov = __shfl_xor(best, o);
      const int oi = __shfl_xor(bi, o);
      if (oi != 0x7fffffff && (bi == 0x7fffffff || ov > best || (ov == best && oi < bi))) {
        best = ov;
        bi = oi;
      }
    }
    if (lane == 0) {
      y[row] = best;
      idx[row] = bi;
    }
  } else {
    float s = 0.0f;
    for (int t = lane; t < L; t += 64) s += xr[t];
#pragma unroll
    for (int o = 32; o > 0; o >>= 1) s += __shfl_xor(s, o);
    if (lane == 0) y[row] = s / (float)L;
  }
}

template <int MODE>
__global__ void pool_time_bwd_kernel(const float* __restrict__ dy, const int* __restrict__ idx,
                                     float* __restrict__ dx, int rows, int L) {
  const size_t n = (size_t)rows * L;
  const float invL = 1.0f / (float)L;
  for (size_t i = blockIdx.x * (size_t)blockDim.x + threadIdx.x; i < n;
       i += (size_t)gridDim.x * blockDim.x) {
    const int row = (int)(i / L);
    const int t = (int)(i - (size_t)row * L);
    dx[i] = MODE == 0 ? (t == idx[row] ? dy[row] : 0.0f) : dy[row] * invL;
  }
}

extern "C" int segan_pool_time_fwd(const float* x, float* y, int* idx, int rows, int L, int mode,
                                   void* stream) {
  SEGAN_REQUIRE(x && y && rows > 0 && L > 0, "pool_time_fwd: bad arguments");
  SEGAN_REQUIRE(mode == 0 || mode == 1, "pool_time_fwd: mode must be 0 (max) or 1 (mean)");
  SEGAN_REQUIRE(mode == 1 || idx, "pool_time_fwd: max pooling needs idx");
  const dim3 grid(ceil_div(rows, 4));
  if (mode == 0)
    hipLaunchKernelGGL(pool_time_kernel<0>, grid, dim3(256), 0, (hipStream_t)stream, x, y, idx,
                       rows, L);
  else
    hipLaunchKernelGGL(pool_time_kernel<1>, grid, dim3(256), 0, (hipStream_t)stream, x, y, idx,
                       rows, L);
  return segan_check_launch("pool_time_fwd");
}

extern "C" int segan_pool_time_bwd(const float* dy, const int* idx, float* dx, int rows, int L,
                                   int mode, void* stream) {
  SEGAN_REQUIRE(dy && dx && rows > 0 && L > 0, "pool_time_bwd: bad arguments");
  SEGAN_REQUIRE(mode == 0 || mode == 1, "pool_time_bwd: mode must be 0 (max) or 1 (mean)");
  SEGAN_REQUIRE(mode == 1 || idx, "pool_time_bwd: max pooling needs idx");
  const size_t n = (size_t)rows * L;
  const int blocks = (int)((n + 255) / 256 > 4096 ? 4096 : (n + 255) / 256);
  if (mode == 0)
    hipLaunchKernelGGL(pool_time_bwd_kernel<0>, dim3(blocks), dim3(256), 0, (hipStream_t)stream,
                       dy, idx, dx, rows, L);
  else
    hipLaunchKernelGGL(pool_time_bwd_kernel<1>, dim3(blocks), dim3(256), 0, (hipStream_t)stream,
                       dy, idx, dx, rows, L);
  return segan_check_launch("pool_time_bwd");
}

__global__ void fill_kernel(float* p, float value, size_t n) {
  for (size_t i = blockIdx.x * (size_t)blockDim.x + threadIdx.x; i < n;
       i += (size_t)gridDim.x * blockDim.x)
    p[i] = value;
}
__global__ void scale_kernel(float* p, float s, size_t n) {
  for (size_t i = blockIdx.x * (size_t)blockDim.x + threadIdx.x; i < n;
       i += (size_t)gridDim.x * blockDim.x)
    p[i] *= s;
}
extern "C" int segan_fill(float* p, float value, int64_t n, void* stream) {
  SEGAN_REQUIRE(p && n > 0, "fill: bad arguments");
  int blocks = (int)((n + 255) / 256 > 4096 ? 4096 : (n + 255) / 256);
  hipLaunchKernelGGL(fill_kernel, dim3(blocks), dim3(256), 0, (hipStream_t)stream, p, value,
                     (size_t)n);
  return segan_check_launch("fill");
}
extern "C" int segan_scale(float* p, float s, int64_t n, void* stream) {
  SEGAN_REQUIRE(p && n > 0, "scale: bad arguments");
  int blocks = (int)((n + 255) / 256 > 4096 ? 4096 : (n + 255) / 256);
  hipLaunchKernelGGL(scale_kernel, dim3(blocks), dim3(256), 0, (hipStream_t)stream, p, s,
                     (size_t)n);
  return segan_check_launch("scale");
}
```

### segan_pytorch_amd/functional.py

```python
import os

import torch

from . import ops
from .ops import ACT_NONE, ACT_TANH, PAD_REFLECT, PAD_ZERO, Src


def grad_buf(p):
    if p.grad is None:
        p.grad = torch.zeros_like(p, memory_format=torch.contiguous_format)
    elif not p.grad.is_contiguous():
        p.grad = p.grad.contiguous()
    return p.grad


def _gb(p, needed=True):
    if p is None or not needed or not p.requires_grad:
        return None
    return grad_buf(p)


def _bn_batch_stats(bn, training):
    return training or bn.running_mean is None or bn.running_var is None


def _bn_train_stats(c, bn, training=True):
    from . import distributed as sdist
    fn = sdist.bn_stats_sync if sdist.sync_bn_enabled() else ops.bn_stats
    track = training and bn.running_mean is not None and bn.running_var is not None
    momentum = 0.0
    if track:
        if bn.num_batches_tracked is not None:
            bn.num_batches_tracked += 1
        if bn.momentum is not None:
            momentum = bn.momentum
        else:
            momentum = 1.0 / float(bn.num_batches_tracked) if bn.num_batches_tracked is not None else 0.0
    return fn(c, bn.weight, bn.bias, bn.eps, momentum, bn.running_mean if track else None,
              bn.running_var if track else None)


def _bn_eval_affine(bn):
    rstd = torch.rsqrt(bn.running_var + bn.eps)
    gamma = bn.weight.detach() if bn.weight is not None else torch.ones_like(rstd)
    beta = bn.bias.detach() if bn.bias is not None else torch.zeros_like(rstd)
    scale = (gamma * rstd).contiguous()
    shift = (beta - bn.running_mean * scale).contiguous()
    return scale, shift, rstd.contiguous()


def _eval_bn_act_bwd(c, bn, scale, shift, rstd, dh, slope, dslope, y_tanh=None, dbias=None):
    if y_tanh is not None:
        g = ops.tanh_bwd(y_tanh, dh, dbias=_gb(bn.bias))
    else:
        v = ops.affine_prelu(c, scale, shift, None)
        g = ops.act_bwd(v, dh, slope=slope, dslope=dslope, dbias=_gb(bn.bias))
    if bn.weight is not None and bn.weight.requires_grad:
        xhat = ops.affine_prelu(c, rstd, (-bn.running_mean * rstd).contiguous(), None)
        grad_buf(bn.weight).add_((g * xhat).sum((0, 2)))
    dc = ops.affine_prelu(g, scale, None, None)
    if dbias is not None:
        ops.act_bwd(dc, dc, dbias=dbias)
    return dc


def _act_bwd_bn(a, dh, slope, bn, dslope, dgamma, dbeta, dbias):
    from . import distributed as sdist
    if sdist.sync_bn_enabled():
        return sdist.act_bwd_bn_sync(a, dh, slope, bn, dslope, dgamma, dbeta, dbias)
    return ops.act_bwd(a, dh, slope=slope, bn=bn, dslope=dslope, dgamma=dgamma, dbeta=dbeta,
                       dbias=dbias)


_WGRAD_OVERLAP = os.environ.get('SEGAN_WGRAD_OVERLAP', '0') == '1'
_side_streams = {}


class _SideStream(object):

    def __init__(self, *tensors):
        flat = []
        for t in tensors:
            if isinstance(t, Src):
                flat.extend((t.t0, t.t1, t.scale, t.shift, t.slope))
            else:
                flat.append(t)
        self.tensors = [t for t in flat if torch.is_tensor(t) and t.is_cuda]
        self.on = _WGRAD_OVERLAP and bool(self.tensors)

    def __enter__(self):
        if not self.on:
            return self
        dev = self.tensors[0].device
        main = torch.cuda.current_stream(dev)
        key = (dev.index, main.cuda_stream)
        side = _side_streams.get(key)
        if side is None:
            side = _side_streams[key] = torch.cuda.Stream(device=dev)
        side.wait_stream(main)
        self.side = side
        self.ctx = torch.cuda.stream(side)
        self.ctx.__enter__()
        return self

    def __exit__(self, *exc):
        if not self.on:
            return False
        self.ctx.__exit__(*exc)
        for t in self.tensors:
            t.record_stream(self.side)
        return False


def _join_side(ref):
    if not _WGRAD_OVERLAP or ref is None or not ref.is_cuda:
        return
    main = torch.cuda.current_stream(ref.device)
    side = _side_streams.get((ref.device.index, main.cuda_stream))
    if side is not None:
        main.wait_stream(side)


def _ready(*mods_or_params):
    from . import distributed as sdist
    if sdist._active is None:
        return
    ps = []
    for m in mods_or_params:
        if m is None:
            continue
        if isinstance(m, torch.nn.Module):
            ps.extend(torch.nn.Module.parameters(m))
        else:
            ps.append(m)
    sdist.grad_ready(*ps)


def _ones(n, ref):
    return torch.ones(n, device=ref.device, dtype=torch.float32)


def _cat(a, b):
    return torch.cat((a.detach().reshape(-1), b.detach().reshape(-1)))


import itertools as _it

_sn_epoch = _it.count(1 << 40)


def _is_sn(mod):
    return hasattr(mod, 'weight_orig')


class _Weights(object):

    def __init__(self):
        self._sn = {}

    def get(self, mod):
        if not _is_sn(mod):
            return mod.weight
        st = self._sn.get(id(mod))
        if st is None:
            dim = 1 if isinstance(mod, torch.nn.ConvTranspose1d) else 0
            w_sn, sigma = ops.snorm_fwd(mod.weight_orig.detach(), mod.weight_u, mod.weight_v, dim,
                                        mod.training)
            w_sn._segan_epoch = next(_sn_epoch)
            st = (w_sn, mod.weight_u.clone(), mod.weight_v.clone(), sigma, dim)
            self._sn[id(mod)] = st
        return st[0]

    @staticmethod
    def param(mod):
        return mod.weight_orig if _is_sn(mod) else mod.weight

    def needs_grad(self, mod):
        return self.param(mod).requires_grad

    def grad_target(self, mod):
        if not _is_sn(mod):
            return grad_buf(mod.weight)
        return torch.zeros_like(self._sn[id(mod)][0])

    def finish(self, mod, tmp):
        if not _is_sn(mod):
            return
        w_sn, u, v, sigma, dim = self._sn[id(mod)]
        ops.snorm_bwd(tmp, mod.weight_orig.detach(), u, v, sigma, dim, grad_buf(mod.weight_orig))


def _skip_conv_bwd(gskip, dsk, src_j, W):
    mod = gskip.skip_k
    kw = mod.kernel_size[0]
    w = W.get(mod)
    if mod.bias is not None and mod.bias.requires_grad:
        ops.act_bwd(dsk, dsk, dbias=grad_buf(mod.bias))
    if W.needs_grad(mod):
        gw = W.grad_target(mod)
        ops.wgrad(Src(dsk), src_j, gw, kw, 1, kw // 2, PAD_ZERO)
        W.finish(mod, gw)
    key = (w.data_ptr(), w._version, ops._weights_epoch, getattr(w, '_segan_epoch', 0))
    cached = gskip.__dict__.get('_wt_cache')
    if cached is None or cached[0] != key:
        wt = w.detach().transpose(0, 1).flip(2).contiguous()
        wt._segan_epoch = next(_sn_epoch)
        cached = (key, wt)
        gskip.__dict__['_wt_cache'] = cached
    return ops.conv1d_fwd(Src(dsk), cached[1], None, 1, pad_mode=PAD_ZERO, padL=kw - 1 - kw // 2,
                          pack=gskip._pack_t)


def _block_norm(blk, c, training):
    bn = getattr(blk, 'norm', None)
    if bn is None:
        return None, None, None
    if _bn_batch_stats(bn, training):
        mean, rstd, scale, shift = _bn_train_stats(c, bn, training)
        return scale, shift, (mean, rstd, bn.weight, bn.bias)
    scale, shift, _rstd = _bn_eval_affine(bn)
    return scale, shift, 'eval'


def _vec2(v0, n0, v1, n1, fill, ref):
    if v0 is None and v1 is None:
        return None
    parts = []
    for v, n in ((v0, n0), (v1, n1)):
        parts.append(v.detach().reshape(-1) if v is not None else
                     torch.full((n,), fill, device=ref.device, dtype=torch.float32))
    return torch.cat(parts)


def _dropout_mask(shape, p, device):
    noise = torch.nn.functional.dropout(torch.ones(shape), p, True)
    return noise.to(device)


class GeneratorFn(torch.autograd.Function):

    @staticmethod
    def forward(ctx, gen, want_hid, x, z, *params):
        x = x.contiguous()
        enc, dec = list(gen.enc_blocks), list(gen.dec_blocks)
        n_enc = len(enc)
        training = gen.training
        a_enc, src_enc, xf_enc, bn_enc = [], [], [], []
        src = Src(x)
        W = _Weights()
        for blk in enc:
            a = ops.conv1d_fwd(src, W.get(blk.conv), blk.conv.bias, blk.stride, pack=blk._pack)
            sc, sh, bnsv = _block_norm(blk, a, training)
            src_enc.append(src)
            a_enc.append(a)
            xf_enc.append((sc, sh))
            bn_enc.append(bnsv)
            src = Src(a, scale=sc, shift=sh, slope=blk.act.weight)
        last = a_enc[-1]
        s_last = enc[-1].act.weight
        sc_l, sh_l = xf_enc[-1]
        if not gen.no_z:
            z = z.contiguous()
            nz, nl = z.shape[1], last.shape[1]
            src = Src(z, last, scale=_vec2(None, nz, sc_l, nl, 1.0, z),
                      shift=_vec2(None, nz, sh_l, nl, 0.0, z), slope=_cat(_ones(nz, z), s_last))
        else:
            src = Src(last, scale=sc_l, shift=sh_l, slope=s_last)
        a_dec, src_dec, xf_dec, bn_dec = [], [], [], []
        skip_saved = {}
        enc_idx = n_enc - 1
        for li, blk in enumerate(dec):
            is_conv = hasattr(blk, 'conv')
            if li > 0:
                prev = a_dec[-1]
                s_prev = dec[li - 1].act.weight
                sc_p, sh_p = xf_dec[-1]
                np_ = prev.shape[1]
                if gen.skip and enc_idx in gen.skips and gen.dec_poolings[li] > 1:
                    gskip = gen.skips[enc_idx]['alpha']
                    aj = a_enc[enc_idx]
                    sc_j, sh_j = xf_enc[enc_idx]
                    nj = aj.shape[1]
                    ones_j = _ones(nj, aj)
                    drop_p = gskip.skip_dropout.p if (training and hasattr(gskip, 'skip_dropout')) \
                        else 0.0
                    a_norm = None
                    if gskip.skip_type == 'conv':
                        kw = gskip.skip_k.kernel_size[0]
                        sk = ops.conv1d_fwd(Src(aj, scale=sc_j, shift=sh_j), W.get(gskip.skip_k),
                                            gskip.skip_k.bias, 1, pad_mode=PAD_ZERO, padL=kw // 2,
                                            pack=gskip._pack)
                        scale_j = ones_j
# ... 58 lines not shown
        hid = None
        if want_hid:
            hid = {}
            for i, blk in enumerate(enc):
                hid['enc_{}'.format(i)] = ops.affine_prelu(a_enc[i], xf_enc[i][0], xf_enc[i][1],
                                                           blk.act.weight)
            if not gen.no_z:
                hid['enc_zc'] = torch.cat((z, hid['enc_{}'.format(n_enc - 1)]), dim=1)
            for i, blk in enumerate(dec):
                if i == len(dec) - 1:
                    hid['dec_{}'.format(i)] = y
                else:
                    hid['dec_{}'.format(i)] = ops.affine_prelu(a_dec[i], xf_dec[i][0],
                                                               xf_dec[i][1], blk.act.weight)
        ctx.mark_non_differentiable(*([] if hid is None else list(hid.values())))
        if hid is None:
            return y
        return (y,) + tuple(hid.values())

    @staticmethod
    def backward(ctx, dy, *unused):
        gen = ctx.gen
        x, z, a_enc, src_enc, xf_enc, bn_enc, a_dec, src_dec, bn_dec, skip_saved, W = ctx.state
        y = ctx.saved_tensors[0]
        a_dec = list(a_dec) if ctx.keep_last else list(a_dec) + [y]
        enc, dec = list(gen.enc_blocks), list(gen.dec_blocks)
        n_enc, n_dec = len(enc), len(dec)
        if dy is None:
            ctx.state = None
            return (None,) * len(ctx.needs_input_grad)
        if 'eval' in bn_enc or 'eval' in bn_dec:
            raise RuntimeError('Generator backward in eval() mode with BatchNorm is not supported; '
                               'call .train()')
        dy = dy.contiguous()
        dh = dy
        dskip = {}
        dh_last_enc = None
        da = None
        for li in range(n_dec - 1, -1, -1):
            blk = dec[li]
            is_conv = hasattr(blk, 'conv')
            mod = blk.conv if is_conv else blk.deconv
            w = W.get(mod)
            K, S = blk.kwidth, blk.stride
            bnsv = bn_dec[li]
            bnm = getattr(blk, 'norm', None)
            if not is_conv and blk.is_tanh:
                if bnsv is None:
                    da = ops.tanh_bwd(a_dec[li], dy, dbias=_gb(mod.bias))
                else:
                    da = _act_bwd_bn(a_dec[li], ops.tanh_bwd(y, dy), None, bnsv, None,
                                     _gb(bnm.weight), _gb(bnm.bias), _gb(mod.bias))
            elif bnsv is None:
                da = ops.act_bwd(a_dec[li], dh, slope=blk.act.weight,
                                 dslope=_gb(blk.act.weight), dbias=_gb(mod.bias))
            else:
                da = _act_bwd_bn(a_dec[li], dh, blk.act.weight, bnsv, _gb(blk.act.weight),
                                 _gb(bnm.weight), _gb(bnm.bias), _gb(mod.bias))
            src = src_dec[li]
            with _SideStream(da, src):
                if W.needs_grad(mod):
                    gw = W.grad_target(mod)
                    if is_conv:
                        ops.wgrad(Src(da), src, gw, K, S, ops.conv_pad(K, S)[0], PAD_REFLECT)
                    else:
                        ops.wgrad(src, Src(da), gw, K, S, ops.deconv_pad(K, S), PAD_ZERO)
                    W.finish(mod, gw)
                _ready(blk)
            if is_conv:
                d_in = ops.conv1d_dgrad(da, w, src.L, S, pack=blk._pack)
                if li == 0:
                    dh_last_enc = d_in if gen.no_z else d_in[:, src.C0:].contiguous()
                else:
                    dh = d_in
            elif li == 0:
                if gen.no_z:
                    _d0, dh_last_enc = ops.deconv1d_dgrad(da, w, S, 0, pack=blk._pack)
                else:
                    _d0, dh_last_enc = ops.deconv1d_dgrad(da, w, S, src.C0, need0=False,
                                                          pack=blk._pack)
            else:
                if src.C1 > 0:
                    dh, dsk = ops.deconv1d_dgrad(da, w, S, src.C0, pack=blk._pack)
                    dskip[n_enc - 1 - li] = dsk
                else:
                    _d0, dh = ops.deconv1d_dgrad(da, w, S, 0, pack=blk._pack)
                    if getattr(src, 'sum_of', False):
                        dskip[n_enc - 1 - li] = dh
        dh = dh_last_enc
        dx = None
        for l in range(n_enc - 1, -1, -1):
            blk = enc[l]
            w = W.get(blk.conv)
            K, S = blk.kwidth, blk.stride
            bnsv = bn_enc[l]
            bnm = getattr(blk, 'norm', None)
            sc, sh = xf_enc[l]
            gskip = gen.skips[l]['alpha'] if (gen.skip and l in gen.skips) else None
            dsk = dskip.get(l)
            mask, a_norm = skip_saved.get(l, (None, None))
            if dsk is not None and mask is not None:
                dsk = ops.scale_mask(dsk, None, mask)
            alpha_p = None
            if gskip is not None and gskip.skip_type == 'conv':
                if dsk is not None:
                    dsk = _skip_conv_bwd(gskip, dsk, Src(a_enc[l], scale=sc, shift=sh), W)
                alpha_v = _ones(a_enc[l].shape[1], a_enc[l]) if dsk is not None else None
                ready_extra = gskip.skip_k
            else:
                alpha_p = gskip.skip_k if gskip is not None else None
                alpha_v = alpha_p if dsk is not None else None
                ready_extra = alpha_p
            if bnsv is None:
                da = ops.act_bwd(a_enc[l], dh, dskip=dsk, slope=blk.act.weight, alpha=alpha_v,
                                 dslope=_gb(blk.act.weight),
                                 dalpha=_gb(alpha_p, dsk is not None),
                                 dbias=_gb(blk.conv.bias))
            elif dsk is None:
                da = _act_bwd_bn(a_enc[l], dh, blk.act.weight, bnsv, _gb(blk.act.weight),
                                 _gb(bnm.weight), _gb(bnm.bias), _gb(blk.conv.bias))
            else:
                if a_norm is None:
                    a_norm = ops.affine_prelu(a_enc[l], sc, sh, None)
                g = ops.act_bwd(a_norm, dh, dskip=dsk, slope=blk.act.weight, alpha=alpha_v,
                                dslope=_gb(blk.act.weight), dalpha=_gb(alpha_p, True))
                da = _act_bwd_bn(a_enc[l], g, None, bnsv, None, _gb(bnm.weight), _gb(bnm.bias),
                                 _gb(blk.conv.bias))
            padL = ops.conv_pad(K, S)[0]
            with _SideStream(da, src_enc[l]):
                if W.needs_grad(blk.conv):
                    gw = W.grad_target(blk.conv)
                    ops.wgrad(Src(da), src_enc[l], gw, K, S, padL, PAD_REFLECT)
                    W.finish(blk.conv, gw)
                _ready(blk, ready_extra)
            if l > 0:
                dh = ops.conv1d_dgrad(da, w, src_enc[l].L, S, pack=blk._pack)
            elif ctx.x_needs:
                dx = ops.conv1d_dgrad(da, w, src_enc[l].L, S, pack=blk._pack)
        _join_side(dy)
        ctx.state = None
        return (None, None, dx, None) + (None,) * (len(ctx.needs_input_grad) - 4)


class DiscriminatorFn(torch.autograd.Function):

    @staticmethod
    def forward(ctx, disc, rolls, x, x1, *params):
        x = x.contiguous()
        blocks = list(disc.enc_blocks)
        training = disc.training
        src = Src(x) if x1 is None else Src(x, x1.contiguous())
        cs, srcs, bns, xfs = [], [], [], []
        W = _Weights()
        for l, blk in enumerate(blocks):
            c = ops.conv1d_fwd(src, W.get(blk.conv), blk.conv.bias, blk.stride, roll=rolls[l],
                               pack=blk._pack)
            srcs.append(src)
            cs.append(c)
            if blk.norm is not None:
                bn = blk.norm
                if _bn_batch_stats(bn, training):
                    mean, rstd, scale, shift = _bn_train_stats(c, bn, training)
                    bns.append((mean, rstd, bn.weight, bn.bias))
                else:
                    scale, shift, _rstd = _bn_eval_affine(bn)
                    bns.append('eval')
                xfs.append((scale, shift))
                src = Src(c, scale=scale, shift=shift, slope=blk.act.weight)
            else:
                bns.append(None)
                xfs.append((None, None))
                src = Src(c, slope=blk.act.weight)
        h = ops.affine_prelu(cs[-1], xfs[-1][0], xfs[-1][1], blocks[-1].act.weight)
        B = h.shape[0]
        fc = disc.fc
        pt = disc.pool_type
        extra = {}
        if pt == 'none':
            hf = h.view(B, -1)
            y1 = ops.linear_fwd(hf, W.get(fc[0]))
            a1 = ops.bias_prelu_rows(y1, fc[0].bias, W.get(fc[1]))
            y2 = ops.linear_fwd(a1, W.get(fc[2]))
            a2 = ops.bias_prelu_rows(y2, fc[2].bias, W.get(fc[3]))
            y3 = ops.linear_fwd(a2, W.get(fc[4]))
            out = ops.bias_prelu_rows(y3, fc[4].bias, None)
            head = (hf, y1, a1, y2, a2, y3)
        else:
            if pt == 'conv':
                pc = ops.conv1d_fwd(Src(h), W.get(disc.pool_conv), disc.pool_conv.bias, 1,
                                    pad_mode=PAD_ZERO, padL=0, pack=disc._pool_pack)
                hp, idx = pc.view(B, -1), None
                extra['avg_conv_h'] = hp
            else:
                hp, idx = ops.pool_time_fwd(h, 'max' if pt == 'gmax' else 'avg')
            y3 = ops.linear_fwd(hp, W.get(fc))
            out = ops.bias_prelu_rows(y3, fc.bias, None)
            head = (h, hp, idx, y3)
        ctx.disc = disc
        ctx.rolls = tuple(rolls)
        ctx.x_needs = x.requires_grad or (x1 is not None and x1.requires_grad)
        ctx.split = None if x1 is None else (x.shape[1], x.requires_grad, x1.requires_grad)
        ctx.state = (cs, srcs, bns, head, W)
        disc._last_fwd = (cs, xfs)
        disc._last_extra = extra
        disc._last_head = head
        return out

    @staticmethod
    def backward(ctx, dout):
        disc = ctx.disc
        cs, srcs, bns, head, W = ctx.state
        blocks = list(disc.enc_blocks)
        fc = disc.fc
        dout = dout.contiguous()
        def lin_wgrad(mod, dy, xin):
            if W.needs_grad(mod):
                gw = W.grad_target(mod)
                ops.linear_wgrad(dy, xin, gw)
                W.finish(mod, gw)

        def prelu_bwd(y, lin, act, dact):
            gs = W.grad_target(act) if W.needs_grad(act) else None
            d = ops.bias_prelu_rows_bwd(y, lin.bias, W.get(act), dact, gs, _gb(lin.bias))
            if gs is not None:
                W.finish(act, gs)
            return d

        if disc.pool_type == 'none':
            hf, y1, a1, y2, a2, y3 = head
            dy3 = ops.bias_prelu_rows_bwd(y3, fc[4].bias, None, dout, None, _gb(fc[4].bias))
            lin_wgrad(fc[4], dy3, a2)
            da2 = ops.linear_dgrad(dy3, W.get(fc[4]))
            dy2 = prelu_bwd(y2, fc[2], fc[3], da2)
            lin_wgrad(fc[2], dy2, a1)
            da1 = ops.linear_dgrad(dy2, W.get(fc[2]))
            dy1 = prelu_bwd(y1, fc[0], fc[1], da1)
            lin_wgrad(fc[0], dy1, hf)
            dh = ops.linear_dgrad(dy1, W.get(fc[0])).view(cs[-1].shape)
            _ready(fc)
        else:
            h, hp, idx, y3 = head
            Lh = h.shape[2]
            dy3 = ops.bias_prelu_rows_bwd(y3, fc.bias, None, dout, None, _gb(fc.bias))
            lin_wgrad(fc, dy3, hp)
            dhp = ops.linear_dgrad(dy3, W.get(fc))
            if disc.pool_type == 'conv':
                pcm = disc.pool_conv
                dpc = dhp.view(h.shape[0], 1, Lh)
                if pcm.bias is not None and pcm.bias.requires_grad:
                    ops.act_bwd(dpc, dpc, dbias=grad_buf(pcm.bias))
                if W.needs_grad(pcm):
                    gw = W.grad_target(pcm)
                    ops.wgrad(Src(dpc), Src(h), gw, 1, 1, 0, PAD_ZERO)
                    W.finish(pcm, gw)
                dh = ops.conv1d_dgrad(dpc, W.get(pcm), Lh, 1, padL=0, pack=disc._pool_pack)
                _ready(fc, pcm)
            else:
                dh = ops.pool_time_bwd(dhp, idx, Lh, 'max' if disc.pool_type == 'gmax' else 'avg')
                _ready(fc)
        dx = None
        for l in range(len(blocks) - 1, -1, -1):
            blk = blocks[l]
            w = W.get(blk.conv)
            K, S = blk.kwidth, blk.stride
            bn = bns[l]
            if bn == 'eval':
                raise RuntimeError('Discriminator backward in eval() mode with BatchNorm is not '
                                   'supported; call .train() (the reference never does this)')
            if bn is not None:
                dc = _act_bwd_bn(cs[l], dh, blk.act.weight, bn, _gb(blk.act.weight), _gb(bn[2]),
                                 _gb(bn[3]), _gb(blk.conv.bias))
            else:
                dc = ops.act_bwd(cs[l], dh, slope=blk.act.weight, dslope=_gb(blk.act.weight),
                                 dbias=_gb(blk.conv.bias))
            padL = ops.conv_pad(K, S)[0]
            with _SideStream(dc, srcs[l]):
                if W.needs_grad(blk.conv):
                    gw = W.grad_target(blk.conv)
                    ops.wgrad(Src(dc), srcs[l], gw, K, S, padL, PAD_REFLECT, roll=ctx.rolls[l])
                    W.finish(blk.conv, gw)
                _ready(blk)
            if l > 0:
                dh = ops.conv1d_dgrad(dc, w, srcs[l].L, S, roll=ctx.rolls[l], pack=blk._pack)
            elif ctx.x_needs:
                dx = ops.conv1d_dgrad(dc, w, srcs[l].L, S, roll=ctx.rolls[l], pack=blk._pack)
        _join_side(dout)
        ctx.state = None
        dx1 = None
        if dx is not None and ctx.split is not None:
            c0, need0, need1 = ctx.split
            dx1 = dx[:, c0:].contiguous() if need1 else None
            dx = dx[:, :c0].contiguous() if need0 else None
        return (None, None, dx, dx1) + (None,) * (len(ctx.needs_input_grad) - 4)


class ConvBlockFn(torch.autograd.Function):

    @staticmethod
    def forward(ctx, blk, x, *params):
        x = x.contiguous()
        src = Src(x)
        W = _Weights()
        c = ops.conv1d_fwd(src, W.get(blk.conv), blk.conv.bias, blk.stride, pack=blk._pack)
        bn_saved = None
        scale = shift = None
        if blk.norm is not None:
            bn = blk.norm
            if _bn_batch_stats(bn, blk.training):
                mean, rstd, scale, shift = _bn_train_stats(c, bn, blk.training)
                bn_saved = (mean, rstd, bn.weight, bn.bias)
            else:
                scale, shift, rstd = _bn_eval_affine(bn)
                bn_saved = ('eval', scale, shift, rstd)
        h = ops.affine_prelu(c, scale, shift, blk.act.weight)
        a = c if blk.norm is None else ops.affine_prelu(c, scale, shift, None)
# ... 197 lines not shown
```

### segan_pytorch_amd/ops.py

```python
import ctypes
import operator

import torch

from . import _lib
from . import layout
from ._lib import ACT_NONE, ACT_TANH, PAD_REFLECT, PAD_ZERO, SeganSrc, check


import os as _os

PREC_FP32, PREC_BF16, PREC_BF16X3 = 0, 1, 3
_PREC_NAMES = {'fp32': PREC_FP32, 'bf16': PREC_BF16, 'bf16x3': PREC_BF16X3}
_precision = _PREC_NAMES[_os.environ.get('SEGAN_PRECISION', 'fp32')]
_EUNSUPPORTED = -3


_deterministic = _os.environ.get('SEGAN_DETERMINISTIC', '0') == '1'


def set_deterministic(on):
    global _deterministic
    _deterministic = bool(on)


def get_deterministic():
    return _deterministic


_ACC_NAMES = ('plain', 'blocked')
_accumulation = _os.environ.get('SEGAN_ACCUMULATION', 'plain')
if _accumulation not in _ACC_NAMES:
    raise ValueError('SEGAN_ACCUMULATION must be one of {}'.format(_ACC_NAMES))
PREC_FP32_BLOCKED = 4


def set_accumulation(mode):
    global _accumulation
    if mode not in _ACC_NAMES:
        raise ValueError('accumulation must be one of {}'.format(_ACC_NAMES))
    _accumulation = mode


def get_accumulation():
    return _accumulation


def _fp32():
    return PREC_FP32_BLOCKED if _accumulation == 'blocked' else PREC_FP32


def set_precision(mode):
    global _precision
    if mode not in _PREC_NAMES:
        raise ValueError('precision must be one of {}'.format(sorted(_PREC_NAMES)))
    _precision = _PREC_NAMES[mode]


def get_precision():
    return [k for k, v in _PREC_NAMES.items() if v == _precision][0]


def _stream():
    return ctypes.c_void_p(torch._C._cuda_getCurrentRawStream(torch._C._cuda_getDevice()))


def _ptr(t):
    if t is None:
        return None
    return ctypes.c_void_p(t.data_ptr())


def _chk(t, name, ndim=None):
    if not isinstance(t, torch.Tensor):
        raise TypeError('{} must be a tensor, got {}'.format(name, type(t)))
    if not t.is_cuda:
        raise RuntimeError(
            '{} is on {}: segan_pytorch_amd runs only on an MI355X (HIP) device; '
            'there is no CPU path'.format(name, t.device))
    if t.dtype != torch.float32:
        raise TypeError('{} must be float32, got {}'.format(name, t.dtype))
    if not t.is_contiguous():
        raise ValueError('{} must be contiguous'.format(name))
    if ndim is not None and t.dim() != ndim:
        raise ValueError('{} must have {} dims, got {}'.format(name, ndim, tuple(t.shape)))
    return t


class Src(object):

    def __init__(self, t0, t1=None, scale=None, shift=None, slope=None):
        _chk(t0, 'src.t0', 3)
        self.t0, self.t1 = t0, t1
        self.C0 = t0.shape[1]
        self.C1 = 0
        if t1 is not None:
            _chk(t1, 'src.t1', 3)
            if t1.shape[0] != t0.shape[0] or t1.shape[2] != t0.shape[2]:
                raise ValueError('src segments disagree: {} vs {}'.format(
                    tuple(t0.shape), tuple(t1.shape)))
            self.C1 = t1.shape[1]
        self.C = self.C0 + self.C1
        for name, v in (('scale', scale), ('shift', shift), ('slope', slope)):
            if v is not None:
                _chk(v, 'src.' + name)
                if v.numel() != self.C:
                    raise ValueError('src.{} has {} entries for {} channels'.format(
                        name, v.numel(), self.C))
        self.scale, self.shift, self.slope = scale, shift, slope
        self.B, self.L = t0.shape[0], t0.shape[2]

    def c_struct(self):
        s = SeganSrc()
        s.p0 = self.t0.data_ptr()
        s.p1 = self.t1.data_ptr() if self.t1 is not None else None
        s.C0, s.C1 = self.C0, self.C1
        s.scale = self.scale.data_ptr() if self.scale is not None else None
        s.shift = self.shift.data_ptr() if self.shift is not None else None
        s.slope = self.slope.data_ptr() if self.slope is not None else None
        return s


_corr_scratch = {}


def _scratch():
    dev = torch._C._cuda_getDevice()
    key = (dev, torch._C._cuda_getCurrentRawStream(dev))
    buf = _corr_scratch.get(key)
    if buf is None:
        nbytes = _lib.load().segan_corr_scratch_bytes()
        buf = torch.empty(nbytes, device=torch.device('cuda', dev), dtype=torch.uint8)
        _corr_scratch[key] = buf
    return ctypes.c_void_p(buf.data_ptr()), buf.numel()


def last_corr_launch():
    arr = (ctypes.c_int * 6)()
    _lib.load().segan_debug_last_corr(arr)
    k = ('kernel', 'workgroups', 'tiles', 'tiles_whole', 'streamk_units', 'xf_mode')
    d = dict(zip(k, list(arr)))
    d['streamk'] = d['streamk_units'] > 0
    return d


def last_wgrad_launch():
    arr = (ctypes.c_int * 6)()
    _lib.load().segan_debug_last_wgrad(arr)
    return dict(zip(('kernel', 'tiles', 'splits', 'chunks_per_split', 'resident_per_cu', 'hi_loads'),
                    list(arr)))


_call_scratch = {}


def _stream_scratch(nbytes, device):
    dev = torch.device(device).index
    if dev is None:
        dev = torch._C._cuda_getDevice()
    key = (dev, torch._C._cuda_getCurrentRawStream(dev))
    buf = _call_scratch.get(key)
    if buf is None or buf.numel() < nbytes:
        buf = None
        _call_scratch.pop(key, None)
        buf = torch.empty(int(nbytes), device=torch.device('cuda', dev), dtype=torch.uint8)
        _call_scratch[key] = buf
    return buf


def set_reserved_slots(n):
    return int(_lib.load().segan_set_reserved_slots(int(n)))


def release_scratch(device=None):
    dev = None if device is None else torch.device(device).index
    for d in (_corr_scratch, _call_scratch):
        for key in [k for k in d if dev is None or k[0] == dev]:
            del d[key]


def scratch_bytes():
    return sum(b.numel() for d in (_corr_scratch, _call_scratch) for b in d.values())


def _bf_scratch(op, B, N, M, L, K, S, pad, device):
    planes = 3 if _precision == PREC_BF16X3 else 1
    nbytes = _lib.load().segan_bf16_scratch_bytes(op, B, N, M, L, K, S, pad, planes)
    if nbytes == 0:
        return None, None, 0
    buf = _stream_scratch(nbytes, device)
    return buf, ctypes.c_void_p(buf.data_ptr()), nbytes


def conv_pad(K, S):
    return layout.conv_pad(K, S)


def deconv_pad(K, S):
    return layout.deconv_pad(K, S)


_weights_epoch = 0


def bump_weights_epoch(params=None):
    global _weights_epoch
    if params is None:
        _weights_epoch += 1
        return
    for p in params:
        p._segan_epoch = getattr(p, '_segan_epoch', 0) + 1


class WeightPack(object):

    def __init__(self):
        self._buf = {}
        self._key = {}

    def _get(self, w, S, pad_t, want):
        _chk(w, 'weight', 3)
        key = (w.data_ptr(), w._version, _weights_epoch, getattr(w, '_segan_epoch', 0),
               tuple(w.shape), S, pad_t)
        if self._key.get(want) == key:
            return self._buf[want]
        lib = _lib.load()
        M, N, K = w.shape
        nbytes = (lib.segan_packed_f_bytes if want == 'f' else lib.segan_packed_t_bytes)(M, N, S)
        if nbytes == 0:
            raise ValueError('unsupported stride {} (must be 1, 2 or 4)'.format(S))
        buf = self._buf.get(want)
        if buf is None or buf.numel() * 4 != nbytes or buf.device != w.device:
            buf = torch.empty(nbytes // 4, device=w.device, dtype=torch.float32)
        check(lib.segan_pack_weights(_ptr(w), _ptr(buf) if want == 'f' else None,
                                     _ptr(buf) if want == 't' else None, M, N, K, S, pad_t,
                                     _stream()), 'pack_weights')
        self._buf[want] = buf
        self._key[want] = key
        return buf

    def f(self, w, S):
        return self._get(w, S, 0, 'f')

    def g(self, w, S):
        _chk(w, 'weight', 3)
        key = (w.data_ptr(), w._version, _weights_epoch, getattr(w, '_segan_epoch', 0),
               tuple(w.shape), S)
        if self._key.get('g') == key:
            return self._buf['g']
        lib = _lib.load()
        M, N, K = w.shape
        nbytes = lib.segan_packed_g_bytes(M, N, S)
        if nbytes == 0:
            raise ValueError('G packing: stride {} not supported'.format(S))
        buf = self._buf.get('g')
        if buf is None or buf.numel() * 4 != nbytes or buf.device != w.device:
            buf = torch.empty(nbytes // 4, device=w.device, dtype=torch.float32)
        check(lib.segan_pack_weights_g(_ptr(w), _ptr(buf), M, N, K, S, _stream()), 'pack_weights_g')
        self._buf['g'] = buf
        self._key['g'] = key
        return buf

    def t(self, w, S, pad_t):
        return self._get(w, S, pad_t, 't')

    def bf(self, w, S, pad_t, tform, planes):
        _chk(w, 'weight', 3)
        want = ('bf', tform, planes)
        key = (w.data_ptr(), w._version, _weights_epoch, getattr(w, '_segan_epoch', 0),
               tuple(w.shape), S, pad_t)
        if self._key.get(want) == key:
            return self._buf[want]
        lib = _lib.load()
        M, N, K = w.shape
        nbytes = lib.segan_packed_bf_bytes(M, N, S, tform, planes)
        if nbytes == 0:
            raise ValueError('unsupported geometry for bf16 packing')
        buf = self._buf.get(want)
        if buf is None or buf.numel() * 2 != nbytes or buf.device != w.device:
            buf = torch.empty(nbytes // 2, device=w.device, dtype=torch.bfloat16)
        check(lib.segan_pack_weights_bf(_ptr(w), _ptr(buf), M, N, K, S, tform, pad_t, planes,
                                        _stream()), 'pack_weights_bf')
        self._buf[want] = buf
        self._key[want] = key
        return buf


def conv1d_fwd(src, w, bias, S, roll=0, pad_mode=PAD_REFLECT, padL=None, pack=None):
    M, N, K = w.shape
    if src.C != N:
        raise ValueError('conv1d_fwd: input has {} channels, weight expects {}'.format(src.C, N))
    B, L = src.B, src.L
    if L % S != 0:
        raise ValueError('conv1d_fwd: length {} not divisible by stride {}'.format(L, S))
    if padL is None:
        padL = conv_pad(K, S)[0]
    out = torch.empty((B, M, L // S), device=w.device, dtype=torch.float32)
    cs = src.c_struct()
    pack = pack or WeightPack()
    lib = _lib.load()
    if _precision and pad_mode == PAD_REFLECT:
        keep, sp, sn = _bf_scratch(0, B, N, M, L, K, S, padL, w.device)
        rc = lib.segan_conv1d_fwd(ctypes.byref(cs), _ptr(pack.bf(w, S, 0, 0, _precision)),
                                  _ptr(bias), _ptr(out), B, N, M, L, K, S, padL, pad_mode, roll,
                                  _precision, sp, sn, _stream())
        if rc != _EUNSUPPORTED:
            check(rc, 'conv1d_fwd')
            return out
    check(lib.segan_conv1d_fwd(ctypes.byref(cs), _ptr(pack.f(w, S)), _ptr(bias), _ptr(out), B, N,
                               M, L, K, S, padL, pad_mode, roll, _fp32(), *_scratch(), _stream()),
          'conv1d_fwd')
    return out


def conv1d_dgrad(da, w, L, S, roll=0, padL=None, pack=None):
    _chk(da, 'da', 3)
    M, N, K = w.shape
    B = da.shape[0]
    if da.shape[1] != M or da.shape[2] * S != L:
        raise ValueError('conv1d_dgrad: da {} inconsistent with weight {} / L {}'.format(
            tuple(da.shape), tuple(w.shape), L))
    if padL is None:
        padL = conv_pad(K, S)[0]
    small = N <= 2
    _chk(w, 'weight', 3)
    pack = pack or WeightPack()
    if not small and not _precision and short_rows_ok(N, M, L, S):
        return conv1d_dgrad_short(da, w, L, S, roll=roll, padL=padL, pack=pack)
    dx = torch.empty((B, N, L), device=da.device, dtype=torch.float32)
    halo = torch.empty((B * N * max(K - 1, 1),), device=da.device, dtype=torch.float32)
    lib = _lib.load()
    if small:
        check(lib.segan_conv1d_dgrad(_ptr(da), None, _ptr(w.detach()), _ptr(dx), _ptr(halo), B, N,
                                     M, L, K, S, padL, roll, PREC_FP32, None, 0, _stream()),
              'conv1d_dgrad')
        return dx
    if _precision:
        keep, sp, sn = _bf_scratch(1, B, N, M, L, K, S, padL, da.device)
        rc = lib.segan_conv1d_dgrad(_ptr(da), _ptr(pack.bf(w, S, 0, 1, _precision)), None, _ptr(dx),
                                    _ptr(halo), B, N, M, L, K, S, padL, roll, _precision, sp, sn,
                                    _stream())
        if rc != _EUNSUPPORTED:
            check(rc, 'conv1d_dgrad')
            return dx
    if short_rows_ok(N, M, L, S):
        return conv1d_dgrad_short(da, w, L, S, roll=roll, padL=padL, pack=pack)
    check(lib.segan_conv1d_dgrad(_ptr(da), _ptr(pack.t(w, S, 0)), None, _ptr(dx), _ptr(halo), B, N,
                                 M, L, K, S, padL, roll, _fp32(), *_scratch(), _stream()),
          'conv1d_dgrad')
    return dx


def conv1d_dgrad_short(da, w, L, S, roll=0, padL=None, pack=None):
    _chk(da, 'da', 3)
    _chk(w, 'weight', 3)
    M, N, K = w.shape
    B = da.shape[0]
    if padL is None:
        padL = conv_pad(K, S)[0]
    dx = torch.empty((B, N, L), device=da.device, dtype=torch.float32)
    pack = pack or WeightPack()
    check(_lib.load().segan_conv1d_dgrad_short(_ptr(da), _ptr(pack.g(w, S)), _ptr(dx), B, N,
                                               M, L, K, S, padL, roll, _stream()),
          'conv1d_dgrad_short')
    return dx


_SHORT_LS = (4, 8, 16, 32, 64)


def short_rows_ok(N, M, L, S):
    return S in (2, 4) and L % S == 0 and (L // S) in _SHORT_LS and N % 4 == 0 and M % 16 == 0


def wgrad(lo, hi, dw, K, S, padL, pad_mode, roll=0):
    _chk(dw, 'dw', 3)
    M, N = lo.C, hi.C
    if tuple(dw.shape) != (M, N, K):
        raise ValueError('wgrad: dw {} != ({}, {}, {})'.format(tuple(dw.shape), M, N, K))
    if lo.B != hi.B or lo.L * S != hi.L:
        raise ValueError('wgrad: lo [{}x{}] / hi [{}x{}] inconsistent for stride {}'.format(
            lo.B, lo.L, hi.B, hi.L, S))
    cl, ch = lo.c_struct(), hi.c_struct()
    lib = _lib.load()
    if _precision != PREC_FP32:
        nbytes = lib.segan_wgrad_scratch_bytes(lo.B, M, N, lo.L, S, _precision, 0)
        scratch = _stream_scratch(nbytes, dw.device)
        rc = lib.segan_wgrad(ctypes.byref(cl), ctypes.byref(ch), _ptr(dw), lo.B, M, N, lo.L, K, S,
                             padL, pad_mode, roll, _precision, 0,
                             ctypes.c_void_p(scratch.data_ptr()) if scratch is not None else None,
                             nbytes if scratch is not None else 0, _stream())
        if rc != -3:
            check(rc, 'wgrad')
            return
    flags = 1 if _deterministic else 0
    lo_plain = lo.t1 is None and lo.scale is None and lo.shift is None and lo.slope is None
    scratch, nbytes = None, 0
    if flags or not lo_plain:
        nbytes = lib.segan_wgrad_scratch_bytes(lo.B, M, N, lo.L, S, PREC_FP32, flags)
        scratch = _stream_scratch(nbytes, dw.device)
    check(lib.segan_wgrad(ctypes.byref(cl), ctypes.byref(ch), _ptr(dw), lo.B, M, N, lo.L, K, S, padL,
                          pad_mode, roll, PREC_FP32, flags,
                          ctypes.c_void_p(scratch.data_ptr()) if scratch is not None else None, nbytes,
                          _stream()), 'wgrad')


def deconv1d_fwd(src, w, bias, S, act=ACT_NONE, pack=None):
    M, N, K = w.shape
    if src.C != M:
        raise ValueError('deconv1d_fwd: input has {} channels, weight expects {}'.format(src.C, M))
    pad = deconv_pad(K, S)
    B, Ls = src.B, src.L
    y = torch.empty((B, N, S * Ls), device=w.device, dtype=torch.float32)
# ... 425 lines not shown


def snorm_bwd(dw_sn, w, u, v, sigma, dim, dw):
    _chk(dw_sn, 'dw_sn')
    _chk(dw, 'dw')
    A, Bd, K = _sn_view(w, dim)
    lib = _lib.load()
    ws = torch.empty(lib.segan_snorm_ws_floats(A, Bd, K, dim), device=w.device, dtype=torch.float32)
    check(lib.segan_snorm_bwd(_ptr(dw_sn), _ptr(w), _ptr(u), _ptr(v), _ptr(sigma), _ptr(dw), _ptr(ws),
                              A, Bd, K, dim, _stream()), 'snorm_bwd')


def pcm16_prep(pcm, first, coef):
    if pcm.dtype != torch.int16 or first.dtype != torch.uint8 or not pcm.is_cuda or not first.is_cuda:
        raise TypeError('pcm16_prep: pcm must be a CUDA int16 tensor and first a CUDA uint8 tensor')
    if pcm.dim() != 3 or pcm.shape[1] != 2 or not pcm.is_contiguous() or first.numel() != pcm.shape[0]:
        raise ValueError('pcm16_prep: pcm must be contiguous [B, 2, T+1], first [B]')
    B, T = pcm.shape[0], pcm.shape[2] - 1
    clean = torch.empty((B, T), device=pcm.device, dtype=torch.float32)
    noisy = torch.empty((B, T), device=pcm.device, dtype=torch.float32)
    check(_lib.load().segan_pcm16_prep(ctypes.c_void_p(pcm.data_ptr()),
                                       ctypes.c_void_p(first.data_ptr()), _ptr(clean), _ptr(noisy),
                                       B, T, float(coef), _stream()), 'pcm16_prep')
    return clean, noisy


def de_emphasize(y, coef):
    _chk(y, 'y')
    T = y.shape[-1]
    x = torch.empty_like(y)
    check(_lib.load().segan_deemphasis(_ptr(y), _ptr(x), y.numel() // T, T, float(coef), _stream()),
          'deemphasis')
    return x


def ssnr(ref, deg, srate=16000, eps=1e-10):
    _chk(ref, 'ref', 2)
    _chk(deg, 'deg', 2)
    if ref.shape != deg.shape:
        raise ValueError('ssnr: shapes differ {} vs {}'.format(tuple(ref.shape), tuple(deg.shape)))
    rows, T = ref.shape
    lib = _lib.load()
    nf = lib.segan_ssnr_frames(T, srate)
    seg = torch.empty((rows, max(nf, 1)), device=ref.device, dtype=torch.float32)
    out = torch.empty((rows, 2), device=ref.device, dtype=torch.float32)
    check(lib.segan_ssnr(_ptr(ref), _ptr(deg), _ptr(seg), _ptr(out), rows, T, srate, float(eps),
                         _stream()), 'ssnr')
    return out[:, 0], out[:, 1], seg[:, :nf]


def _quality_frames(fn, what, ref, deg, srate):
    _chk(ref, 'ref', 2)
    _chk(deg, 'deg', 2)
    if ref.shape != deg.shape:
        raise ValueError('{}: shapes differ {} vs {}'.format(what, tuple(ref.shape), tuple(deg.shape)))
    rows, T = ref.shape
    nf = _lib.load().segan_ssnr_frames(T, srate)
    dist = torch.empty((rows, max(nf, 1)), device=ref.device, dtype=torch.float64)
    check(fn(_ptr(ref), _ptr(deg), _ptr(dist), rows, T, srate, _stream()), what)
    return dist[:, :nf]


def wss(ref, deg, srate=16000):
    return _quality_frames(_lib.load().segan_wss, 'wss', ref, deg, srate)


def llr(ref, deg, srate=16000):
    return _quality_frames(_lib.load().segan_llr, 'llr', ref, deg, srate)


STOI_SRATES = (4000, 48000)
STOI_BANDS = 15


def _stoi_srate(srate):
    srate_in = srate
    try:
        srate = None if isinstance(srate, bool) else operator.index(srate)
    except TypeError:
        srate = None
    if srate is None or not STOI_SRATES[0] <= srate <= STOI_SRATES[1]:
        raise ValueError('stoi: srate must be an integer from {} to {} Hz, got {!r}'.format(
            STOI_SRATES[0], STOI_SRATES[1], srate_in))
    return srate


def stoi_plan(srate):
    srate = _stoi_srate(srate)
    lib = _lib.load()
    pq, n, bands = (ctypes.c_int * 2)(), ctypes.c_int(), (ctypes.c_int * (2 * STOI_BANDS))()
    check(lib.segan_stoi_plan(srate, pq, ctypes.byref(n), None, 0, None), 'stoi_plan')
    taps = torch.empty(n.value, dtype=torch.float64)
    check(lib.segan_stoi_plan(srate, pq, ctypes.byref(n), _ptr(taps), n.value, bands), 'stoi_plan')
    return pq[0], pq[1], taps, torch.tensor(list(bands), dtype=torch.int64).view(STOI_BANDS, 2)


def _stoi_lengths(lengths, rows, T, device):
    lens = torch.as_tensor(lengths).detach().cpu()
    if lens.dim() != 1 or lens.numel() != rows or lens.dtype.is_floating_point or lens.dtype in (
            torch.bool, torch.complex64, torch.complex128):
        raise ValueError('stoi: lengths must hold {} integers, got {}'.format(rows, lengths))
    if rows and (int(lens.min()) < 0 or int(lens.max()) > T):
        raise ValueError('stoi: lengths must lie in 0 .. {}, got {}'.format(T, lens.tolist()))
    return lens.to(dtype=torch.int32).to(device)


def stoi_stages(ref, deg, srate=16000, lengths=None):
    _chk(ref, 'ref', 2)
    _chk(deg, 'deg', 2)
    if ref.shape != deg.shape:
        raise ValueError('stoi: shapes differ {} vs {}'.format(tuple(ref.shape), tuple(deg.shape)))
    srate = _stoi_srate(srate)
    rows, T = ref.shape
    lens = None if lengths is None else _stoi_lengths(lengths, rows, T, ref.device)
    lib = _lib.load()
    dims = (ctypes.c_int * 5)()
    check(lib.segan_stoi_dims(T, srate, dims), 'stoi')
    Ly, F, Lc, Fb, S = list(dims)
    f64 = dict(device=ref.device, dtype=torch.float64)
    i32 = dict(device=ref.device, dtype=torch.int32)
    xr = torch.empty((2, rows, max(Ly, 1)), **f64)
    energy = torch.empty((rows, max(F, 1)), **f64)
    mask = torch.empty((rows, max(F, 1)), **i32)
    kept = torch.empty((rows, max(F, 1)), **i32)
    count = torch.empty(rows, **i32)
    xs = torch.empty((2, rows, max(Lc, 1)), **f64)
    env = torch.empty((2, rows, STOI_BANDS, max(Fb, 1)), **f64)
    rho = torch.empty((rows, max(S, 1), STOI_BANDS), **f64)
    d = torch.empty(rows, **f64)
    check(lib.segan_stoi(_ptr(ref), _ptr(deg), _ptr(lens), rows, T, srate, _ptr(xr[0]), _ptr(xr[1]),
                         _ptr(energy), _ptr(mask), _ptr(kept), _ptr(count), _ptr(xs[0]),
                         _ptr(xs[1]), _ptr(env[0]), _ptr(env[1]), _ptr(rho), _ptr(d), _stream()),
          'stoi')
    return dict(xr=xr[0, :, :Ly], yr=xr[1, :, :Ly], energy=energy[:, :F], mask=mask[:, :F],
                kept=kept[:, :F], count=count, xs=xs[0, :, :Lc], ys=xs[1, :, :Lc],
                X=env[0, :, :, :Fb], Y=env[1, :, :, :Fb], rho=rho[:, :S], d=d,
                dims=(Ly, F, Lc, Fb, S))


def stoi(ref, deg, srate=16000, lengths=None):
    return stoi_stages(ref, deg, srate, lengths)['d']


def rmsprop_step(p, g, sq, lr, alpha, eps):
    check(_lib.load().segan_rmsprop_step(_ptr(p), _ptr(g), _ptr(sq), lr, alpha, eps, p.numel(),
                                         _stream()), 'rmsprop_step')


def adam_step(p, g, m, v, lr, beta1, beta2, eps, step):
    check(_lib.load().segan_adam_step(_ptr(p), _ptr(g), _ptr(m), _ptr(v), lr, beta1, beta2, eps,
                                      step, p.numel(), _stream()), 'adam_step')


def fill_(t, value):
    _chk(t, 't')
    check(_lib.load().segan_fill(_ptr(t), float(value), t.numel(), _stream()), 'fill')
    return t


def scale_(t, s):
    _chk(t, 't')
    check(_lib.load().segan_scale(_ptr(t), float(s), t.numel(), _stream()), 'scale')
    return t


def comm_unique_id():
    lib = _lib.load()
    buf = ctypes.create_string_buffer(lib.segan_comm_id_bytes())
    check(lib.segan_comm_unique_id(buf), 'comm_unique_id')
    return buf.raw


class Comm(object):

    def __init__(self, world, rank, unique_id):
        lib = _lib.load()
        if len(unique_id) != lib.segan_comm_id_bytes():
            raise ValueError('Comm: unique id must be {} bytes'.format(lib.segan_comm_id_bytes()))
        h = ctypes.c_void_p()
        check(lib.segan_comm_init(ctypes.byref(h), int(world), int(rank), unique_id), 'comm_init')
        self._h, self.world, self.rank = h, int(world), int(rank)

    def _s(self, stream):
        return ctypes.c_void_p((stream or torch.cuda.current_stream()).cuda_stream)

    def allreduce(self, t, scale=1.0, stream=None):
        _chk(t, 't')
        check(_lib.load().segan_allreduce(self._h, _ptr(t), t.numel(), float(scale), self._s(stream)),
              'allreduce')
        return t

    def broadcast(self, t, root=0, stream=None):
        _chk(t, 't')
        check(_lib.load().segan_broadcast(self._h, _ptr(t), t.numel(), int(root), self._s(stream)),
              'broadcast')
        return t

    def allgather(self, send, stream=None):
        _chk(send, 'send')
        recv = torch.empty((self.world,) + tuple(send.shape), device=send.device, dtype=torch.float32)
        check(_lib.load().segan_allgather(self._h, _ptr(send), _ptr(recv), send.numel(),
                                          self._s(stream)), 'allgather')
        return recv

    def destroy(self):
        if self._h is not None:
            check(_lib.load().segan_comm_destroy(self._h), 'comm_destroy')
            self._h = None
```

Baseline: 3571.

## Batch weight repacking, BN counter bumps and fuse act-bwd reductions to cut launches

Adds a table-driven pack kernel that repacks every registered weight layout in one launch after the optimizer step, a single kernel that increments all BatchNorm num_batches_tracked counters, and a fused BN act-backward path where phase 3 folds the cross-split reduction into the apply kernel. It also caches ones tensors and batches the loads in the split-reduction loops. The aim is to cut per-step kernel launch and Python overhead. The costs are registry bookkeeping via weakrefs, eager repacking of weights that may not be used next step, and some redundant reduction work per block.

```diff
diff --git a/include/segan_hip.h b/include/segan_hip.h
--- a/include/segan_hip.h
+++ b/include/segan_hip.h
@@ -8,7 +8,7 @@
 extern "C" {
 #endif
 
-#define SEGAN_ABI_VERSION 16
+#define SEGAN_ABI_VERSION 17
 
 #define SEGAN_PAD_REFLECT 0
 #define SEGAN_PAD_ZERO 1
@@ -36,6 +36,18 @@
 
 int segan_pack_weights(const float* w, float* wf, float* wt, int M, int N, int K, int S,
                        int pad_t, void* stream);
+
+#define SEGAN_PACK_F 0
+#define SEGAN_PACK_T 1
+#define SEGAN_PACK_G 2
+typedef struct segan_pack_job {
+  const float* w;
+  float* dst;
+  int32_t M, N, K, S;
+  int32_t pad_t;
+  int32_t layout;
+} segan_pack_job;
+int segan_pack_weights_table(const segan_pack_job* jobs, int njobs, void* stream);
 
 #define SEGAN_PREC_FP32 0
 #define SEGAN_PREC_BF16 1
@@ -108,6 +120,10 @@
                            const float* bn_beta, const float* totals, float* da, float* dbias,
                            float* ws, int B, int C, int L, double count_total, void* stream);
 
+int segan_set_step_fusion(int on);
+
+int segan_bump_counters(int64_t* const* counters, int n, void* stream);
+
 int segan_tanh_bwd(const float* y, const float* dy, const float* clean, float l1_scale, float* da,
                    float* dbias, float* ws, int B, int C, int L, void* stream);
 
diff --git a/segan_pytorch_amd/_lib.py b/segan_pytorch_amd/_lib.py
--- a/segan_pytorch_amd/_lib.py
+++ b/segan_pytorch_amd/_lib.py
@@ -9,7 +9,15 @@
 PAD_ZERO = 1
 ACT_NONE = 0
 ACT_TANH = 1
-ABI_VERSION = 16
+ABI_VERSION = 17
+
+
+class SeganPackJob(Structure):
+    _fields_ = [('w', c_void_p), ('dst', c_void_p), ('M', c_int32), ('N', c_int32), ('K', c_int32),
+                ('S', c_int32), ('pad_t', c_int32), ('layout', c_int32)]
+
+
+PACK_F, PACK_T, PACK_G = 0, 1, 2
 
 
 class SeganSrc(Structure):
@@ -27,6 +35,9 @@
     'segan_packed_f_bytes': (c_size_t, [c_int, c_int, c_int]),
     'segan_packed_t_bytes': (c_size_t, [c_int, c_int, c_int]),
     'segan_pack_weights': (c_int, [_P, _P, _P, c_int, c_int, c_int, c_int, c_int, _P]),
+    'segan_pack_weights_table': (c_int, [POINTER(SeganPackJob), c_int, _P]),
+    'segan_set_step_fusion': (c_int, [c_int]),
+    'segan_bump_counters': (c_int, [POINTER(c_void_p), c_int, _P]),
     'segan_packed_bf_bytes': (c_size_t, [c_int, c_int, c_int, c_int, c_int]),
     'segan_pack_weights_bf': (c_int, [_P, _P, c_int, c_int, c_int, c_int, c_int, c_int, c_int, _P]),
     'segan_corr_scratch_bytes': (c_size_t, []),
diff --git a/segan_pytorch_amd/csrc/segan_conv.hip b/segan_pytorch_amd/csrc/segan_conv.hip
--- a/segan_pytorch_amd/csrc/segan_conv.hip
+++ b/segan_pytorch_amd/csrc/segan_conv.hip
@@ -1058,19 +1058,6 @@
       }
     }
     __syncthreads();
-  }
-}
-
-__global__ void pack_g_kernel(const float* __restrict__ w, float* __restrict__ wg, int M, int N,
-                              int K, int S) {
-  const size_t total = (size_t)M * N * 32;
-  const int U = 32 / S;
-  for (size_t i = blockIdx.x * (size_t)blockDim.x + threadIdx.x; i < total;
-       i += (size_t)gridDim.x * blockDim.x) {
-    const int c = (int)(i & 31);
-    const size_t mn = i >> 5;
-    const int k = S * (c % U) + c / U;
-    wg[i] = k < K ? w[mn * K + k] : 0.0f;
   }
 }
 
@@ -1551,22 +1538,6 @@
          K - S - padL < L;
 }
 
-extern "C" size_t segan_packed_g_bytes(int M, int N, int S) {
-  if (!stride_ok(S) || M <= 0 || N <= 0) return 0;
-  return (size_t)M * N * 32 * sizeof(float);
-}
-
-extern "C" int segan_pack_weights_g(const float* w, float* wg, int M, int N, int K, int S,
-                                    void* stream) {
-  SEGAN_REQUIRE(w && wg && M > 0 && N > 0, "pack_weights_g: bad arguments");
-  SEGAN_REQUIRE(stride_ok(S) && K >= 1 && K <= 32, "pack_weights_g: stride in {1,2,4}, K <= 32");
-  const size_t total = (size_t)M * N * 32;
-  const int blocks = (int)((total + 255) / 256 > 8192 ? 8192 : (total + 255) / 256);
-  hipLaunchKernelGGL(pack_g_kernel, dim3(blocks), dim3(256), 0, (hipStream_t)stream, w, wg, M, N, K,
-                     S);
-  return segan_check_launch("pack_weights_g");
-}
-
 extern "C" int segan_conv1d_dgrad_short(const float* da, const float* wg, float* dx, int B, int N,
                                         int M, int L, int K, int S, int padL, int roll,
                                         void* stream) {
diff --git a/segan_pytorch_amd/csrc/segan_pack.hip b/segan_pytorch_amd/csrc/segan_pack.hip
--- a/segan_pytorch_amd/csrc/segan_pack.hip
+++ b/segan_pytorch_amd/csrc/segan_pack.hip
@@ -1,11 +1,10 @@
 #include "segan_conv_shared.h"
 
-__global__ __launch_bounds__(256) void pack_f_kernel(const float* __restrict__ w,
-                                                     float* __restrict__ wf, int M, int N, int K,
-                                                     int S, int U, int pitch, int rows, int pair) {
-  __shared__ float t[64][33];
-  const int n = blockIdx.y;
-  const int m0 = blockIdx.x * 64;
+__device__ __forceinline__ void pack_f_tile(const float* __restrict__ w, float* __restrict__ wf,
+                                            int M, int N, int K, int S, int U, int pitch, int rows,
+                                            int pair, int bx, int by, float (*t)[33]) {
+  const int n = by;
+  const int m0 = bx * 64;
   const int tid = threadIdx.x;
   {
     float v[8];
@@ -36,13 +35,18 @@
   }
 }
 
-__global__ __launch_bounds__(256) void pack_t_kernel(const float* __restrict__ w,
-                                                     float* __restrict__ wt, int M, int N, int K,
-                                                     int S, int U, int NP, int pad, int pitch,
-                                                     int rows) {
+__global__ __launch_bounds__(256) void pack_f_kernel(const float* __restrict__ w,
+                                                     float* __restrict__ wf, int M, int N, int K,
+                                                     int S, int U, int pitch, int rows, int pair) {
   __shared__ float t[64][33];
-  const int m = blockIdx.y;
-  const int n0 = blockIdx.x * 64;
+  pack_f_tile(w, wf, M, N, K, S, U, pitch, rows, pair, blockIdx.x, blockIdx.y, t);
+}
+
+__device__ __forceinline__ void pack_t_tile(const float* __restrict__ w, float* __restrict__ wt,
+                                            int M, int N, int K, int S, int U, int NP, int pad,
+                                            int pitch, int rows, int bx, int by, float (*t)[33]) {
+  const int m = by;
+  const int n0 = bx * 64;
   const int tid = threadIdx.x;
   {
     float v[8];
@@ -68,6 +72,71 @@
     const int row = m * U + up;
     const int n = n0 + nl;
     if (row < rows && n < NP) wt[(size_t)row * pitch + r * NP + n] = t[nl][k];
+  }
+}
+
+__global__ __launch_bounds__(256) void pack_t_kernel(const float* __restrict__ w,
+                                                     float* __restrict__ wt, int M, int N, int K,
+                                                     int S, int U, int NP, int pad, int pitch,
+                                                     int rows) {
+  __shared__ float t[64][33];
+  pack_t_tile(w, wt, M, N, K, S, U, NP, pad, pitch, rows, blockIdx.x, blockIdx.y, t);
+}
+
+__device__ __forceinline__ void pack_g_elems(const float* __restrict__ w, float* __restrict__ wg,
+                                             int M, int N, int K, int S, size_t first,
+                                             size_t stride) {
+  const size_t total = (size_t)M * N * 32;
+  const int U = 32 / S;
+  for (size_t i = first; i < total; i += stride) {
+    const int c = (int)(i & 31);
+    const size_t mn = i >> 5;
+    const int k = S * (c % U) + c / U;
+    wg[i] = k < K ? w[mn * K + k] : 0.0f;
+  }
+}
+
+__global__ void pack_g_kernel(const float* __restrict__ w, float* __restrict__ wg, int M, int N,
+                              int K, int S) {
+  pack_g_elems(w, wg, M, N, K, S, blockIdx.x * (size_t)blockDim.x + threadIdx.x,
+               (size_t)gridDim.x * blockDim.x);
+}
+
+static int pack_g_blocks(int M, int N) {
+  const size_t total = (size_t)M * N * 32;
+  return (int)((total + 255) / 256 > 8192 ? 8192 : (total + 255) / 256);
+}
+
+#define PACK_TABLE_JOBS 64
+struct PackJob {
+  const float* w;
+  float* dst;
+  int M, N;
+  int blk0;
+  int gx;
+  int pitch, rows, NP;
+  unsigned char K, S, pad, layout, pair;
+};
+struct PackTable {
+  PackJob job[PACK_TABLE_JOBS];
+  int njobs;
+};
+static_assert(sizeof(PackTable) <= 4096, "the pack table travels as a kernel argument");
+
+__global__ __launch_bounds__(256) void pack_table_kernel(const PackTable tb) {
+  __shared__ float t[64][33];
+  int j = 0;
+  while (j + 1 < tb.njobs && (int)blockIdx.x >= tb.job[j + 1].blk0) ++j;
+  const PackJob& q = tb.job[j];
+  const int local = (int)blockIdx.x - q.blk0;
+  const int M = q.M, N = q.N, K = q.K, S = q.S, U = 32 / q.S;
+  if (q.layout == SEGAN_PACK_F) {
+    pack_f_tile(q.w, q.dst, M, N, K, S, U, q.pitch, q.rows, q.pair, local % q.gx, local / q.gx, t);
+  } else if (q.layout == SEGAN_PACK_T) {
+    pack_t_tile(q.w, q.dst, M, N, K, S, U, q.NP, q.pad, q.pitch, q.rows, local % q.gx,
+                local / q.gx, t);
+  } else {
+    pack_g_elems(q.w, q.dst, M, N, K, S, (size_t)local * 256 + threadIdx.x, (size_t)q.gx * 256);
   }
 }
 
@@ -102,3 +171,69 @@
   }
   return segan_check_launch("pack_weights");
 }
+
+extern "C" size_t segan_packed_g_bytes(int M, int N, int S) {
+  if (!stride_ok(S) || M <= 0 || N <= 0) return 0;
+  return (size_t)M * N * 32 * sizeof(float);
+}
+
+extern "C" int segan_pack_weights_g(const float* w, float* wg, int M, int N, int K, int S,
+                                    void* stream) {
+  SEGAN_REQUIRE(w && wg && M > 0 && N > 0, "pack_weights_g: bad arguments");
+  SEGAN_REQUIRE(stride_ok(S) && K >= 1 && K <= 32, "pack_weights_g: stride in {1,2,4}, K <= 32");
+  hipLaunchKernelGGL(pack_g_kernel, dim3(pack_g_blocks(M, N)), dim3(256), 0, (hipStream_t)stream, w,
+                     wg, M, N, K, S);
+  return segan_check_launch("pack_weights_g");
+}
+
+extern "C" int segan_pack_weights_table(const segan_pack_job* jobs, int njobs, void* stream) {
+  SEGAN_REQUIRE(njobs >= 0 && (jobs != nullptr || njobs == 0), "pack_weights_table: bad table");
+  for (int i = 0; i < njobs; ++i) {
+    const segan_pack_job& q = jobs[i];
+    SEGAN_REQUIRE(q.w && q.dst, "pack_weights_table: job %d: NULL pointer", i);
+    SEGAN_REQUIRE(stride_ok(q.S), "pack_weights_table: job %d: stride %d not in {1,2,4}", i, q.S);
+    SEGAN_REQUIRE(q.K >= 1 && q.K <= 32, "pack_weights_table: job %d: kernel width %d not in [1,32]",
+                  i, q.K);
+    SEGAN_REQUIRE(q.M > 0 && q.N > 0, "pack_weights_table: job %d: bad channel counts %d,%d", i, q.M,
+                  q.N);
+    SEGAN_REQUIRE(q.layout == SEGAN_PACK_F || q.layout == SEGAN_PACK_T || q.layout == SEGAN_PACK_G,
+                  "pack_weights_table: job %d: unknown layout %d", i, q.layout);
+    SEGAN_REQUIRE(q.pad_t >= 0 && q.pad_t < 256, "pack_weights_table: job %d: bad padding %d", i,
+                  q.pad_t);
+  }
+  if (njobs == 0) return SEGAN_OK;
+  for (int i0 = 0; i0 < njobs; i0 += PACK_TABLE_JOBS) {
+    PackTable tb = {};
+    tb.njobs = njobs - i0 < PACK_TABLE_JOBS ? njobs - i0 : PACK_TABLE_JOBS;
+    int blocks = 0;
+    for (int i = 0; i < tb.njobs; ++i) {
+      const segan_pack_job& q = jobs[i0 + i];
+      PackJob& d = tb.job[i];
+      d.w = q.w; d.dst = q.dst; d.M = q.M; d.N = q.N;
+      d.K = (unsigned char)q.K; d.S = (unsigned char)q.S; d.pad = (unsigned char)q.pad_t;
+      d.layout = (unsigned char)q.layout;
+      d.blk0 = blocks;
+      const int U = 32 / q.S;
+      d.pitch = d.rows = d.NP = 0;
+      d.pair = 0;
+      if (q.layout == SEGAN_PACK_F) {
+        d.pitch = f_pitch(q.M);
+        d.rows = f_rows(q.N);
+        d.pair = (unsigned char)f_pair(q.N, q.K);
+        d.gx = d.pitch / 64;
+        blocks += d.gx * ceil_div(d.rows, 32);
+      } else if (q.layout == SEGAN_PACK_T) {
+        d.NP = t_np(q.N, q.S);
+        d.pitch = t_pitch(q.N, q.S);
+        d.rows = t_rows(q.M, q.S);
+        d.gx = ceil_div(d.NP, 64);
+        blocks += d.gx * ceil_div(d.rows, U);
+      } else {
+        d.gx = pack_g_blocks(q.M, q.N);
+        blocks += d.gx;
+      }
+    }
+    hipLaunchKernelGGL(pack_table_kernel, dim3(blocks), dim3(256), 0, (hipStream_t)stream, tb);
+  }
+  return segan_check_launch("pack_weights_table");
+}
diff --git a/segan_pytorch_amd/csrc/segan_pointwise.hip b/segan_pytorch_amd/csrc/segan_pointwise.hip
--- a/segan_pytorch_amd/csrc/segan_pointwise.hip
+++ b/segan_pytorch_amd/csrc/segan_pointwise.hip
@@ -1,6 +1,8 @@
 #include "segan_common.h"
+#include <stdlib.h>
 
 #define PW_THREADS 256
+#define PW_AHEAD 8
 
 static int pw_nsplit(int B, int C, int L) {
   int ns = ceil_div(2048, C);
@@ -136,15 +138,24 @@
   const int c = blockIdx.x * blockDim.x + threadIdx.x;
   if (c >= C) return;
   double n = 0.0, mean = 0.0, m2 = 0.0;
-  for (int s = 0; s < nsplit; ++s) {
-    const float* w = ws + ((size_t)s * C + c) * 3;
-    const double nb = w[0], mb = w[1], qb = w[2];
-    if (nb <= 0.0) continue;
-    const double tot = n + nb;
-    const double d = mb - mean;
-    mean += d * nb / tot;
-    m2 += qb + d * d * n * nb / tot;
-    n = tot;
+  for (int s0 = 0; s0 < nsplit; s0 += PW_AHEAD) {
+    float v[PW_AHEAD][3];
+#pragma unroll
+    for (int j = 0; j < PW_AHEAD; ++j) {
+      const float* w = ws + ((size_t)min(s0 + j, nsplit - 1) * C + c) * 3;
+      v[j][0] = w[0]; v[j][1] = w[1]; v[j][2] = w[2];
+    }
+#pragma unroll
+    for (int j = 0; j < PW_AHEAD; ++j) {
+      if (s0 + j >= nsplit) break;
+      const double nb = v[j][0], mb = v[j][1], qb = v[j][2];
+      if (nb <= 0.0) continue;
+      const double tot = n + nb;
+      const double d = mb - mean;
+      mean += d * nb / tot;
+      m2 += qb + d * d * n * nb / tot;
+      n = tot;
+    }
   }
   const double var = n > 0 ? m2 / n : 0.0;
   const float rstd = (float)(1.0 / sqrt(var + (double)eps));
@@ -300,7 +311,26 @@
   float* ws;
   int B, C, L, nsplit;
   float inv_count;
+  float* dslope;
+  float* dgamma;
+  float* dbeta;
 };
+
+static int g_step_fusion = -1;
+static int step_fusion() {
+  int v = __atomic_load_n(&g_step_fusion, __ATOMIC_RELAXED);
+  if (v < 0) {
+    const char* e = getenv("SEGAN_STEP_FUSION");
+    v = (e && e[0] == '0' && e[1] == 0) ? 0 : 1;
+    __atomic_store_n(&g_step_fusion, v, __ATOMIC_RELAXED);
+  }
+  return v;
+}
+extern "C" int segan_set_step_fusion(int on) {
+  const int prev = step_fusion();
+  __atomic_store_n(&g_step_fusion, on ? 1 : 0, __ATOMIC_RELAXED);
+  return prev;
+}
 
 template <int PHASE>
 __global__ void act_bwd_kernel(const ActBwdArgs p) {
@@ -322,6 +352,27 @@
     const float* tot = p.ws + (size_t)p.nsplit * p.C * 4 + (size_t)c * 2;
     dbeta_m = tot[0] * p.inv_count;
     dgamma_m = tot[1] * p.inv_count;
+  }
+  if (PHASE == 3) {
+    float s0 = 0.f, s1 = 0.f, s2 = 0.f;
+    const int lane = threadIdx.x & 63;
+    for (int sb = 0; sb < p.nsplit; sb += 64) {
+      const int nl = min(64, p.nsplit - sb);
+      const float* w = p.ws + ((size_t)(sb + min(lane, nl - 1)) * p.C + c) * 4;
+      const float v0 = w[0], v1 = w[1], v2 = w[2];
+      for (int j = 0; j < nl; ++j) {
+        s0 += __shfl(v0, j, 64);
+        s1 += __shfl(v1, j, 64);
+        s2 += __shfl(v2, j, 64);
+      }
+    }
+    dbeta_m = __fmul_rn(s1, p.inv_count);
+    dgamma_m = __fmul_rn(s2, p.inv_count);
+    if (blockIdx.y == 0 && threadIdx.x == 0) {
+      if (p.dslope) p.dslope[c] += s0;
+      if (p.dbeta) p.dbeta[c] += s1;
+      if (p.dgamma) p.dgamma[c] += s2;
+    }
   }
   float r[3] = {0.f, 0.f, 0.f};
   const bool has_skip = p.dskip != nullptr;
@@ -383,9 +434,13 @@
   block_sum<3>(r, sm);
   if (threadIdx.x == 0) {
     float* w = p.ws + ((size_t)blockIdx.y * p.C + c) * 4;
-    w[0] = r[0];
-    w[1] = r[1];
-    w[2] = r[2];
+    if (PHASE == 3) {
+      w[3] = r[0];
+    } else {
+      w[0] = r[0];
+      w[1] = r[1];
+      w[2] = r[2];
+    }
   }
 }
 
@@ -395,11 +450,20 @@
   const int c = blockIdx.x * blockDim.x + threadIdx.x;
   if (c >= p.C) return;
   float s0 = 0.f, s1 = 0.f, s2 = 0.f;
-  for (int s = 0; s < p.nsplit; ++s) {
-    const float* w = p.ws + ((size_t)s * p.C + c) * 4;
-    s0 += w[0];
-    s1 += w[1];
-    s2 += w[2];
+  for (int sb = 0; sb < p.nsplit; sb += PW_AHEAD) {
+    float v[PW_AHEAD][3];
+#pragma unroll
+    for (int j = 0; j < PW_AHEAD; ++j) {
+      const float* w = p.ws + ((size_t)min(sb + j, p.nsplit - 1) * p.C + c) * 4;
+      v[j][0] = w[PHASE == 3 ? 3 : 0]; v[j][1] = w[1]; v[j][2] = w[2];
+    }
+#pragma unroll
+    for (int j = 0; j < PW_AHEAD; ++j) {
+      if (sb + j >= p.nsplit) break;
+      s0 += v[j][0];
+      s1 += v[j][1];
+      s2 += v[j][2];
+    }
   }
   if (PHASE == 0) {
     if (dslope) dslope[c] += s0;
@@ -435,8 +499,14 @@
   p.da = da; p.ws = ws; p.B = B; p.C = C; p.L = L;
   p.nsplit = pw_nsplit(B, C, L);
   p.inv_count = 1.0f / ((float)B * (float)L);
+  p.dslope = dslope; p.dgamma = dgamma; p.dbeta = dbeta;
   const dim3 grid(C, p.nsplit), fgrid(ceil_div(C, 64));
-  if (!bn_mean) {
+  if (bn_mean && step_fusion()) {
+    hipLaunchKernelGGL(act_bwd_kernel<1>, grid, dim3(PW_THREADS), 0, st, p);
+    hipLaunchKernelGGL(act_bwd_kernel<3>, grid, dim3(PW_THREADS), 0, st, p);
+    hipLaunchKernelGGL(act_bwd_final_kernel<3>, fgrid, dim3(64), 0, st, p, dslope, dalpha, dgamma,
+                       dbeta, dbias);
+  } else if (!bn_mean) {
     hipLaunchKernelGGL(act_bwd_kernel<0>, grid, dim3(PW_THREADS), 0, st, p);
     hipLaunchKernelGGL(act_bwd_final_kernel<0>, fgrid, dim3(64), 0, st, p, dslope, dalpha, dgamma,
                        dbeta, dbias);
@@ -465,6 +535,7 @@
   p.da = nullptr; p.ws = ws; p.B = B; p.C = C; p.L = L;
   p.nsplit = pw_nsplit(B, C, L);
   p.inv_count = 1.0f / ((float)B * (float)L);
+  p.dslope = p.dgamma = p.dbeta = nullptr;
   hipLaunchKernelGGL(act_bwd_kernel<1>, dim3(C, p.nsplit), dim3(PW_THREADS), 0, st, p);
   hipLaunchKernelGGL(act_bwd_final_kernel<1>, dim3(ceil_div(C, 64)), dim3(64), 0, st, p, dslope,
                      (float*)nullptr, dgamma, dbeta, (float*)nullptr);
@@ -490,6 +561,7 @@
   p.da = da; p.ws = ws; p.B = B; p.C = C; p.L = L;
   p.nsplit = pw_nsplit(B, C, L);
   p.inv_count = (float)(1.0 / count_total);
+  p.dslope = p.dgamma = p.dbeta = nullptr;
   if (hipMemcpyAsync(ws + (size_t)p.nsplit * C * 4, totals, (size_t)C * 2 * sizeof(float),
                      hipMemcpyDeviceToDevice, st) != hipSuccess) {
     segan_set_error("act_bwd_bn_apply: copy of the totals failed");
@@ -531,7 +603,16 @@
   const int c = blockIdx.x * blockDim.x + threadIdx.x;
   if (c >= C) return;
   float s = 0.f;
-  for (int k = 0; k < nsplit; ++k) s += ws[(size_t)k * C + c];
+  for (int k0 = 0; k0 < nsplit; k0 += 2 * PW_AHEAD) {
+    float v[2 * PW_AHEAD];
+#pragma unroll
+    for (int j = 0; j < 2 * PW_AHEAD; ++j) v[j] = ws[(size_t)min(k0 + j, nsplit - 1) * C + c];
+#pragma unroll
+    for (int j = 0; j < 2 * PW_AHEAD; ++j) {
+      if (k0 + j >= nsplit) break;
+      s += v[j];
+    }
+  }
   out[c] += s;
 }
 
@@ -585,14 +666,26 @@
   if (c < cols) {
     const float bs = bias ? bias[c] : 0.0f;
     const float sl = slope ? slope[c] : 1.0f;
-    for (int r = rg; r < rows; r += 4) {
-      const size_t i = (size_t)r * cols + c;
-      const float v = x[i] + bs;
-      const float g = dy[i];
-      const float d = g * (v > 0.f ? 1.0f : sl);
-      s_sl += g * (v > 0.f ? 0.0f : v);
-      s_b += d;
-      dx[i] = d;
+    for (int r0 = rg; r0 < rows; r0 += 4 * PW_AHEAD) {
+      float xv[PW_AHEAD], gv[PW_AHEAD];
+#pragma unroll
+      for (int j = 0; j < PW_AHEAD; ++j) {
+        const int r = min(r0 + 4 * j, rows - 1);
+        xv[j] = x[(size_t)r * cols + c];
+        gv[j] = dy[(size_t)r * cols + c];
+      }
+#pragma unroll
+      for (int j = 0; j < PW_AHEAD; ++j) {
+        const int r = r0 + 4 * j;
+        if (r >= rows) break;
+        const size_t i = (size_t)r * cols + c;
+        const float v = xv[j] + bs;
+        const float g = gv[j];
+        const float d = g * (v > 0.f ? 1.0f : sl);
+        s_sl += g * (v > 0.f ? 0.0f : v);
+        s_b += d;
+        dx[i] = d;
+      }
     }
   }
   sm[0][rg][cl] = s_sl;
@@ -900,6 +993,28 @@
        i += (size_t)gridDim.x * blockDim.x)
     p[i] *= s;
 }
+#define BUMP_TABLE 32
+struct BumpTable {
+  long long* p[BUMP_TABLE];
+  int n;
+};
+__global__ void bump_counters_kernel(const BumpTable t) {
+  if ((int)threadIdx.x < t.n) *t.p[threadIdx.x] += 1;
+}
+
+extern "C" int segan_bump_counters(int64_t* const* counters, int n, void* stream) {
+  SEGAN_REQUIRE(n >= 0 && (counters || n == 0), "bump_counters: bad arguments");
+  for (int i = 0; i < n; ++i) SEGAN_REQUIRE(counters[i], "bump_counters: counter %d is NULL", i);
+  if (n == 0) return SEGAN_OK;
+  for (int i0 = 0; i0 < n; i0 += BUMP_TABLE) {
+    BumpTable t = {};
+    t.n = n - i0 < BUMP_TABLE ? n - i0 : BUMP_TABLE;
+    for (int i = 0; i < t.n; ++i) t.p[i] = (long long*)counters[i0 + i];
+    hipLaunchKernelGGL(bump_counters_kernel, dim3(1), dim3(64), 0, (hipStream_t)stream, t);
+  }
+  return segan_check_launch("bump_counters");
+}
+
 extern "C" int segan_fill(float* p, float value, int64_t n, void* stream) {
   SEGAN_REQUIRE(p && n > 0, "fill: bad arguments");
   int blocks = (int)((n + 255) / 256 > 4096 ? 4096 : (n + 255) / 256);
diff --git a/segan_pytorch_amd/functional.py b/segan_pytorch_amd/functional.py
--- a/segan_pytorch_amd/functional.py
+++ b/segan_pytorch_amd/functional.py
@@ -24,13 +24,20 @@
     return training or bn.running_mean is None or bn.running_var is None
 
 
-def _bn_train_stats(c, bn, training=True):
+def _bump_bn_counters(bns, training):
+    ops.bump_counters([bn.num_batches_tracked for bn in bns
+                       if training and bn.running_mean is not None and bn.running_var is not None
+                       and bn.num_batches_tracked is not None])
+    return True
+
+
+def _bn_train_stats(c, bn, training=True, bumped=False):
     from . import distributed as sdist
     fn = sdist.bn_stats_sync if sdist.sync_bn_enabled() else ops.bn_stats
     track = training and bn.running_mean is not None and bn.running_var is not None
     momentum = 0.0
     if track:
-        if bn.num_batches_tracked is not None:
+        if bn.num_batches_tracked is not None and not bumped:
             bn.num_batches_tracked += 1
         if bn.momentum is not None:
             momentum = bn.momentum
@@ -136,8 +143,15 @@
     sdist.grad_ready(*ps)
 
 
+_ones_cache = {}
+
+
 def _ones(n, ref):
-    return torch.ones(n, device=ref.device, dtype=torch.float32)
+    key = (n, ref.device)
+    v = _ones_cache.get(key)
+    if v is None:
+        v = _ones_cache[key] = torch.ones(n, device=ref.device, dtype=torch.float32)
+    return v
 
 
 def _cat(a, b):
@@ -502,6 +516,8 @@
         src = Src(x) if x1 is None else Src(x, x1.contiguous())
         cs, srcs, bns, xfs = [], [], [], []
         W = _Weights()
+        bumped = _bump_bn_counters([blk.norm for blk in blocks if blk.norm is not None and
+                                    _bn_batch_stats(blk.norm, training)], training)
         for l, blk in enumerate(blocks):
             c = ops.conv1d_fwd(src, W.get(blk.conv), blk.conv.bias, blk.stride, roll=rolls[l],
                                pack=blk._pack)
@@ -510,7 +526,7 @@
             if blk.norm is not None:
                 bn = blk.norm
                 if _bn_batch_stats(bn, training):
-                    mean, rstd, scale, shift = _bn_train_stats(c, bn, training)
+                    mean, rstd, scale, shift = _bn_train_stats(c, bn, training, bumped=bumped)
                     bns.append((mean, rstd, bn.weight, bn.bias))
                 else:
                     scale, shift, _rstd = _bn_eval_affine(bn)
diff --git a/segan_pytorch_amd/ops.py b/segan_pytorch_amd/ops.py
--- a/segan_pytorch_amd/ops.py
+++ b/segan_pytorch_amd/ops.py
@@ -1,5 +1,6 @@
 import ctypes
 import operator
+import weakref
 
 import torch
 
@@ -44,6 +45,21 @@
 
 def get_accumulation():
     return _accumulation
+
+
+_step_fusion = _os.environ.get('SEGAN_STEP_FUSION', '1') != '0'
+
+
+def set_step_fusion(on):
+    global _step_fusion
+    prev = _step_fusion
+    _step_fusion = bool(on)
+    _lib.load().segan_set_step_fusion(1 if _step_fusion else 0)
+    return prev
+
+
+def get_step_fusion():
+    return _step_fusion
 
 
 def _fp32():
@@ -210,6 +226,58 @@
         return
     for p in params:
         p._segan_epoch = getattr(p, '_segan_epoch', 0) + 1
+    if _step_fusion:
+        _repack(params)
+
+
+_PACK_LAYOUT = {'f': _lib.PACK_F, 't': _lib.PACK_T, 'g': _lib.PACK_G}
+_pack_registry = {}
+
+
+def _pack_holders(w):
+    ent = _pack_registry.get(id(w))
+    if ent is None or ent[0]() is not w:
+        wid = id(w)
+
+        def gone(ref, wid=wid):
+            if _pack_registry.get(wid, (None,))[0] is ref:
+                del _pack_registry[wid]
+        ent = (weakref.ref(w, gone), {})
+        _pack_registry[wid] = ent
+    return ent[1]
+
+
+def _repack(params):
+    jobs = []
+    for p in params:
+        ent = _pack_registry.get(id(p))
+        if ent is None or ent[0]() is not p or not p.is_cuda:
+            continue
+        reg = ent[1]
+        for ent in list(reg):
+            pack, want, S, pad_t = reg[ent]
+            buf = pack._buf.get(want)
+            if (not pack._used.get(want) or buf is None or buf.device != p.device or
+                    pack._shape.get(want) != tuple(p.shape) or p.dim() != 3 or
+                    p.dtype != torch.float32 or not p.is_contiguous()):
+                del reg[ent]
+                continue
+            jobs.append((p, pack, want, S, pad_t, buf))
+    if not jobs:
+        return
+    dev = jobs[0][0].device
+    if any(j[0].device != dev for j in jobs):
+        return
+    table = (_lib.SeganPackJob * len(jobs))()
+    for q, (p, pack, want, S, pad_t, buf) in zip(table, jobs):
+        q.w, q.dst = p.data_ptr(), buf.data_ptr()
+        q.M, q.N, q.K = p.shape
+        q.S, q.pad_t, q.layout = S, pad_t, _PACK_LAYOUT[want]
+    with torch.cuda.device(dev):
+        check(_lib.load().segan_pack_weights_table(table, len(jobs), _stream()), 'pack_weights_table')
+    for p, pack, want, S, pad_t, buf in jobs:
+        pack._key[want] = pack._mkkey(p, want, S, pad_t)
+        pack._used[want] = False
 
 
 class WeightPack(object):
@@ -217,12 +285,26 @@
     def __init__(self):
         self._buf = {}
         self._key = {}
+        self._used = {}
+        self._shape = {}
+
+    @staticmethod
+    def _mkkey(w, want, S, pad_t):
+        key = (w.data_ptr(), w._version, _weights_epoch, getattr(w, '_segan_epoch', 0),
+               tuple(w.shape), S)
+        return key if want == 'g' else key + (pad_t,)
+
+    def _note(self, w, want, S, pad_t):
+        self._used[want] = True
+        self._shape[want] = tuple(w.shape)
+        if w.is_cuda:
+            _pack_holders(w)[(id(self), want)] = (self, want, S, pad_t)
 
     def _get(self, w, S, pad_t, want):
         _chk(w, 'weight', 3)
-        key = (w.data_ptr(), w._version, _weights_epoch, getattr(w, '_segan_epoch', 0),
-               tuple(w.shape), S, pad_t)
+        key = self._mkkey(w, want, S, pad_t)
         if self._key.get(want) == key:
+            self._used[want] = True
             return self._buf[want]
         lib = _lib.load()
         M, N, K = w.shape
@@ -237,6 +319,7 @@
                                      _stream()), 'pack_weights')
         self._buf[want] = buf
         self._key[want] = key
+        self._note(w, want, S, pad_t)
         return buf
 
     def f(self, w, S):
@@ -244,9 +327,9 @@
 
     def g(self, w, S):
         _chk(w, 'weight', 3)
-        key = (w.data_ptr(), w._version, _weights_epoch, getattr(w, '_segan_epoch', 0),
-               tuple(w.shape), S)
+        key = self._mkkey(w, 'g', S, 0)
         if self._key.get('g') == key:
+            self._used['g'] = True
             return self._buf['g']
         lib = _lib.load()
         M, N, K = w.shape
@@ -259,6 +342,7 @@
         check(lib.segan_pack_weights_g(_ptr(w), _ptr(buf), M, N, K, S, _stream()), 'pack_weights_g')
         self._buf['g'] = buf
         self._key['g'] = key
+        self._note(w, 'g', S, 0)
         return buf
 
     def t(self, w, S, pad_t):
@@ -990,6 +1074,22 @@
                                       step, p.numel(), _stream()), 'adam_step')
 
 
+def bump_counters(counters):
+    counters = list(counters)
+    if not counters:
+        return
+    dev = counters[0].device
+    if not (_step_fusion and all(t.is_cuda and t.device == dev and t.dtype == torch.int64 and
+                                 t.numel() == 1 for t in counters)) or \
+            len(set(t.data_ptr() for t in counters)) != len(counters):
+        for t in counters:
+            t += 1
+        return
+    arr = (ctypes.c_void_p * len(counters))(*[t.data_ptr() for t in counters])
+    with torch.cuda.device(dev):
+        check(_lib.load().segan_bump_counters(arr, len(counters), _stream()), 'bump_counters')
+
+
 def fill_(t, value):
     _chk(t, 't')
     check(_lib.load().segan_fill(_ptr(t), float(value), t.numel(), _stream()), 'fill')
```

Result: no change. 3595 (median of 6 runs) (+0.7%).
